# mstksg/tensor-ops

Measured on AMD Instinct MI355X. Metric: gradTOp steps/sec (ffLayer MNIST 784->256->10) + gmul TFLOP/s vs roofline, higher is better.
Workload: dtype f32

## Files before the change

### tensor-ops_amd/csrc/gemm_small.hip

```cpp
#include "common.hpp"

#include <type_traits>

namespace to {

typedef float f32x16 __attribute__((ext_vector_type(16)));

template <class S>
struct SmallArgsT {
  const S* A;
  const S* B;
  S* C;
  const S* Cin;
  int M, N, K;
  long a_sm, a_sk, b_sk, b_sn, c_sm;
  long a_sb, b_sb, c_sb;
  int a_vec, b_vec;
  unsigned a_bytes, b_bytes;
  int tiles_n;
  int tiles_m;
  int tile_order;
  int kper;
  S alpha, beta;
  const S* bias;
  const S* dact;
  int act;
  int dact_kind;
  S* rowsum;
  const S* rowsum_in;
  S rowsum_alpha;
  int rowsum_acc;
  int loss_rows;
  const S* target;
  S* loss_out;
  const S* tail_w;
  const S* tail_h;
  S* tail_out;
  int tail_n;
#ifdef TOPS_AB_KNOBS
  long long* dbg;
#endif
};

#ifdef TOPS_AB_KNOBS
#define SM_STAMP(i) do { if (stamp_on) g.dbg[i] = wall_clock64(); } while (0)
#else
#define SM_STAMP(i) do { } while (0)
#endif


template <class G>
__device__ __forceinline__ void tile_of(const G& g, int bid, int& tile_m, int& tile_n) {
  if (g.tile_order) {
    const int T = g.tiles_m * g.tiles_n, x = bid & 7, q = T >> 3, r = T & 7;
    bid = (x < r ? x * (q + 1) : r * (q + 1) + (x - r) * q) + (bid >> 3);
  }
  if (g.tile_order == 2) {
    tile_n = bid / g.tiles_m;
    tile_m = bid - tile_n * g.tiles_m;
  } else {
    tile_m = bid / g.tiles_n;
    tile_n = bid - tile_m * g.tiles_n;
  }
}

__device__ __forceinline__ float tanh_s(float x) { return tanhf(x); }
__device__ __forceinline__ double tanh_s(double x) { return tanh(x); }
__device__ __forceinline__ float exp_s(float x) { return expf(x); }
__device__ __forceinline__ double exp_s(double x) { return exp(x); }
__device__ __forceinline__ float log_s(float x) { return logf(x); }
__device__ __forceinline__ double log_s(double x) { return log(x); }
__device__ __forceinline__ float max_s(float a, float b) { return fmaxf(a, b); }
__device__ __forceinline__ double max_s(double a, double b) { return fmax(a, b); }

template <int OFF>
__device__ __forceinline__ float xor16(float x) {
  const int v = __float_as_int(x);
  if constexpr (OFF == 1) return __int_as_float(__builtin_amdgcn_update_dpp(v, v, 0xB1, 0xF, 0xF, false));
  else if constexpr (OFF == 2) return __int_as_float(__builtin_amdgcn_update_dpp(v, v, 0x4E, 0xF, 0xF, false));
  else if constexpr (OFF == 8) return __int_as_float(__builtin_amdgcn_update_dpp(v, v, 0x128, 0xF, 0xF, false));
  else {
    static_assert(OFF == 4, "xor 8, 4, 2 or 1");
    const int up = __builtin_amdgcn_update_dpp(v, v, 0x104, 0xF, 0x5, false);
    return __int_as_float(__builtin_amdgcn_update_dpp(up, v, 0x114, 0xF, 0xA, false));
  }
}
template <int OFF>
__device__ __forceinline__ double xor16(double x) { return __shfl_xor(x, OFF, 64); }

template <class S, int AMODE, int BMODE, int NW, int TS, int ONESHOT = 0, bool EXT = false, int PARTS = 0, bool STAG = false, int TAILK = 0>
__device__ __forceinline__ void gemm_small_body(const SmallArgsT<S>& g, const int bid, const long bz, S* ext_lds = nullptr,
                                                const int tid_in = -1) {
  constexpr int ES = (int)sizeof(S);
  static_assert(ES == 4 || TS == 16, "the fp64 matrix instruction is 16x16x4");
  constexpr int KG = (TS == 32) ? 2 : 4;
  constexpr int NR = (TS == 32) ? 16 : 4;
  constexpr int CK = 4 * KG;
  typedef S accv __attribute__((ext_vector_type(NR)));
  S (*red)[NR][64];
  S (*rsum)[64];
  S* dzs;
  if constexpr (EXT) {
    red = reinterpret_cast<S (*)[NR][64]>(ext_lds);
    rsum = reinterpret_cast<S (*)[64]>(ext_lds + NW * NR * 64);
    dzs = ext_lds + NW * NR * 64 + NW * 64;
  } else {
    __shared__ S red_s[NW][NR][64];
    __shared__ S rsum_s[NW][64];
    __shared__ S dzs_s[TS == 16 ? 16 * 17 : 1];
    red = red_s;
    rsum = rsum_s;
    dzs = dzs_s;
  }
  const int tid = tid_in >= 0 ? tid_in : (int)threadIdx.x, lane = tid & 63, wave = tid >> 6;
  const int l31 = lane & (TS - 1), half = lane / TS;
#ifdef TOPS_AB_KNOBS
  const bool stamp_on = g.dbg && bid == 0 && tid == 0;
#endif
  SM_STAMP(0);
  int tile_m, tile_n;
  tile_of(g, bid, tile_m, tile_n);
  const long m = (long)tile_m * TS + l31, n = (long)tile_n * TS + l31;
  const bool mv = m < g.M, nv = n < g.N;

  accv acc;
#pragma unroll
  for (int r = 0; r < NR; ++r) acc[r] = S(0);
  S asum = S(0);

  const int kbeg = wave * g.kper;
  int kend = kbeg + g.kper;
  if (kend > g.K) kend = g.K;

  constexpr int ST = ONESHOT ? ONESHOT : 4;
  S a0[ST][4], b0[ST][4];
  const __amdgpu_buffer_rsrc_t ra = __builtin_amdgcn_make_buffer_rsrc(
      const_cast<S*>(g.A), 0, g.a_bytes, 0x00020000);
  const __amdgpu_buffer_rsrc_t rb = __builtin_amdgcn_make_buffer_rsrc(
      const_cast<S*>(g.B), 0, g.b_bytes, 0x00020000);
  const int a_base = (int)((bz * g.a_sb + (mv ? m : 0) * g.a_sm) * ES);
  const int b_base = (int)((bz * g.b_sb + (nv ? n : 0) * g.b_sn) * ES);
  const int a_sk4 = (int)g.a_sk * ES, b_sk4 = (int)g.b_sk * ES;
  auto sel = [](bool ok, int off) { const int msk = -(int)ok; return (off & msk) | (0x7fffffff & ~msk); };
  typedef unsigned int u32x4 __attribute__((ext_vector_type(4)));
  typedef unsigned int u32x2 __attribute__((ext_vector_type(2)));
  auto ld1 = [&](__amdgpu_buffer_rsrc_t r, int off) -> S {
    if constexpr (ES == 4) {
      return __uint_as_float(__builtin_amdgcn_raw_buffer_load_b32(r, off, 0, 0));
    } else {
      const u32x2 v = __builtin_amdgcn_raw_buffer_load_b64(r, off, 0, 0);
      return __hiloint2double((int)v.y, (int)v.x);
    }
  };
  auto ld4 = [&](__amdgpu_buffer_rsrc_t r, bool ok, int off, S (&d)[4]) {
    if constexpr (ES == 4) {
      const u32x4 v = __builtin_amdgcn_raw_buffer_load_b128(r, sel(ok, off), 0, 0);
      d[0] = __uint_as_float(v.x); d[1] = __uint_as_float(v.y);
      d[2] = __uint_as_float(v.z); d[3] = __uint_as_float(v.w);
    } else {
      const u32x4 v = __builtin_amdgcn_raw_buffer_load_b128(r, sel(ok, off), 0, 0);
      const u32x4 w = __builtin_amdgcn_raw_buffer_load_b128(r, sel(ok, off + 16), 0, 0);
      d[0] = __hiloint2double((int)v.y, (int)v.x); d[1] = __hiloint2double((int)v.w, (int)v.z);
      d[2] = __hiloint2double((int)w.y, (int)w.x); d[3] = __hiloint2double((int)w.w, (int)w.z);
    }
  };
  auto load_stage = [&](S (&a)[ST][4], S (&b)[ST][4], int k0) {
#pragma unroll
    for (int c = 0; c < ST; ++c) {
      const int kb = k0 + CK * c + 4 * half;
      if (AMODE == 0 && g.a_vec) {
        ld4(ra, mv & (kb < kend), a_base + kb * ES, a[c]);
      } else {
#pragma unroll
        for (int j = 0; j < 4; ++j) a[c][j] = ld1(ra, sel(mv & (kb + j < kend), a_base + (kb + j) * a_sk4));
      }
      if (BMODE == 1 && g.b_vec) {
        ld4(rb, nv & (kb < kend), b_base + kb * ES, b[c]);
      } else {
#pragma unroll
        for (int j = 0; j < 4; ++j) b[c][j] = ld1(rb, sel(nv & (kb + j < kend), b_base + (kb + j) * b_sk4));
      }
    }
  };
  auto mma_stage = [&](const S (&a)[ST][4], const S (&b)[ST][4]) {
#pragma unroll
    for (int c = 0; c < ST; ++c)
#pragma unroll
      for (int j = 0; j < 4; ++j) {
        if constexpr (ES == 8) acc = __builtin_amdgcn_mfma_f64_16x16x4f64(a[c][j], b[c][j], acc, 0, 0, 0);
        else if constexpr (TS == 32) acc = __builtin_amdgcn_mfma_f32_32x32x2f32(a[c][j], b[c][j], acc, 0, 0, 0);
        else acc = __builtin_amdgcn_mfma_f32_16x16x4f32(a[c][j], b[c][j], acc, 0, 0, 0);
        asum += a[c][j];
      }
  };
  constexpr int CP = PARTS ? ST / PARTS : ST;
  static_assert(PARTS == 0 || (ONESHOT && ST % PARTS == 0), "PARTS divides the one-shot batch");
  auto load_part = [&](auto part, int k0) {
    constexpr int p = decltype(part)::value;
#pragma unroll
    for (int c = p * CP; c < (p + 1) * CP; ++c) {
      const int kb = k0 + CK * c + 4 * half;
      if (AMODE == 0 && g.a_vec) {
        ld4(ra, mv & (kb < kend), a_base + kb * ES, a0[c]);
      } else {
#pragma unroll
        for (int j = 0; j < 4; ++j) a0[c][j] = ld1(ra, sel(mv & (kb + j < kend), a_base + (kb + j) * a_sk4));
      }
      if (BMODE == 1 && g.b_vec) {
        ld4(rb, nv & (kb < kend), b_base + kb * ES, b0[c]);
      } else {
#pragma unroll
        for (int j = 0; j < 4; ++j) b0[c][j] = ld1(rb, sel(nv & (kb + j < kend), b_base + (kb + j) * b_sk4));
      }
      __builtin_amdgcn_sched_barrier(0);
    }
  };
  auto mma_part = [&](auto part) {
    constexpr int p = decltype(part)::value;
#pragma unroll
    for (int c = p * CP; c < (p + 1) * CP; ++c) {
#pragma unroll
      for (int j = 0; j < 4; ++j) {
        if constexpr (ES == 8) acc = __builtin_amdgcn_mfma_f64_16x16x4f64(a0[c][j], b0[c][j], acc, 0, 0, 0);
        else if constexpr (TS == 32) acc = __builtin_amdgcn_mfma_f32_32x32x2f32(a0[c][j], b0[c][j], acc, 0, 0, 0);
        else acc = __builtin_amdgcn_mfma_f32_16x16x4f32(a0[c][j], b0[c][j], acc, 0, 0, 0);
      }
      __builtin_amdgcn_sched_barrier(0);
#pragma unroll
      for (int j = 0; j < 4; ++j) asum += a0[c][j];
      __builtin_amdgcn_sched_barrier(0);
    }
  };
  auto row16 = [&](int kg, int r) { return ES == 8 ? kg + 4 * r : 4 * kg + r; };
  constexpr int NRW = (NR + NW - 1) / NW;
  S* Cb = g.C + bz * g.c_sb;
  const S* Ci = g.Cin ? g.Cin + bz * g.c_sb : nullptr;
  const S* Hd = g.dact ? g.dact + bz * g.c_sb : nullptr;
  S pf_ci[NRW], pf_hd[NRW], pf_bias = S(0);
  {
    const long col = (long)tile_n * TS + l31;
    if (g.bias && col < g.N) pf_bias = g.bias[col];
#pragma unroll
    for (int i = 0; i < NRW; ++i) {
      const int r = wave + i * NW;
      const int lrow = (TS == 32) ? (r & 3) + 8 * (r >> 2) + 4 * half : row16(half, r);
      const long row = (long)tile_m * TS + lrow;
      const bool ok = r < NR && row < g.M && col < g.N;
      pf_ci[i] = (Ci && ok) ? Ci[row * g.c_sm + col] : S(0);
      pf_hd[i] = (Hd && ok) ? Hd[row * g.c_sm + col] : S(0);
    }
  }
  constexpr int SK = CK * ST;
  SM_STAMP(1);
  if constexpr (ONESHOT) {
    if constexpr (PARTS == 0) {
      if (kbeg < kend) {
        load_stage(a0, b0, kbeg);
#ifdef TOPS_AB_KNOBS
        if (stamp_on) { SM_STAMP(2); __builtin_amdgcn_s_waitcnt(0x0F70); SM_STAMP(3); }
#endif
        mma_stage(a0, b0);
      }
    } else if (kbeg < kend) {
      if constexpr (STAG) {
        const int lvl = __builtin_amdgcn_readfirstlane(wave) >> 2;
        if (lvl == 0) __builtin_amdgcn_s_setprio(3);
        else if (lvl == 1) __builtin_amdgcn_s_setprio(2);
        else if (lvl == 2) __builtin_amdgcn_s_setprio(1);
      }
      load_part(std::integral_constant<int, 0>{}, kbeg);
      auto stage = [&](auto part) {
        constexpr int p = decltype(part)::value;
        if constexpr (p + 1 < PARTS) load_part(std::integral_constant<int, p + 1>{}, kbeg);
        if constexpr (STAG && p == (PARTS >= 2 ? PARTS - 2 : 0)) __builtin_amdgcn_s_setprio(0);
        __builtin_amdgcn_sched_barrier(0);
        if constexpr (p == 0) SM_STAMP(2);
        mma_part(part);
        __builtin_amdgcn_sched_barrier(0);
        if constexpr (p == 0) SM_STAMP(3);
      };
      stage(std::integral_constant<int, 0>{});
      if constexpr (PARTS > 1) stage(std::integral_constant<int, 1>{});
      if constexpr (PARTS > 2) stage(std::integral_constant<int, 2>{});
      if constexpr (PARTS > 3) stage(std::integral_constant<int, 3>{});
      if constexpr (PARTS > 4) {
        stage(std::integral_constant<int, 4>{});
        stage(std::integral_constant<int, 5>{});
        stage(std::integral_constant<int, 6>{});
        stage(std::integral_constant<int, 7>{});
      }
      static_assert(PARTS == 1 || PARTS == 2 || PARTS == 4 || PARTS == 8, "one, two, four or eight parts");
    }
  } else {
    S a1[ST][4], b1[ST][4];
    if (kbeg < kend) load_stage(a0, b0, kbeg);
    for (int k0 = kbeg; k0 < kend; k0 += 2 * SK) {
      if (k0 + SK < kend) load_stage(a1, b1, k0 + SK);
      mma_stage(a0, b0);
      if (k0 + SK < kend) {
        if (k0 + 2 * SK < kend) load_stage(a0, b0, k0 + 2 * SK);
        mma_stage(a1, b1);
      }
    }
  }

  S tl_bw[2][4], tl_hv[2][4];
  if constexpr (TS == 16) {
    if (g.loss_rows && g.tail_out) {
      const int l15 = lane & 15, kg = lane >> 4;
      const int ntiles = (g.tail_n + 15) / 16;
#pragma unroll
      for (int u = 0; u < 2; ++u) {
        const int t = wave + u * NW;
        const long col = (long)t * 16 + l15;
        const bool cv = t < ntiles && col < g.tail_n;
#pragma unroll
        for (int st = 0; st < 4; ++st) {
          const int k = 4 * st + kg;
          tl_bw[u][st] = (cv && k < g.N) ? g.tail_w[(long)k * g.tail_n + col] : S(0);
        }
#pragma unroll
        for (int r = 0; r < 4; ++r) {
          const long row = (long)tile_m * 16 + row16(kg, r);
          tl_hv[u][r] = (cv && row < g.M) ? g.tail_h[row * g.tail_n + col] : S(0);
        }
      }
    }
  }
#pragma unroll
  for (int r = 0; r < NR; ++r) red[wave][r][lane] = acc[r];
  rsum[wave][lane] = asum;
  SM_STAMP(4);
  __syncthreads();
  SM_STAMP(5);
  if (g.rowsum && tile_n == 0 && wave == 0 && lane < TS) {
    S v = S(0);
#pragma unroll
    for (int w = 0; w < NW; ++w)
#pragma unroll
      for (int q = 0; q < KG; ++q) v += rsum[w][lane + q * TS];
    const long row = (long)tile_m * TS + lane;
    if (row < g.M) g.rowsum[bz * g.M + row] = g.rowsum_acc ? g.rowsum_in[bz * g.M + row] + g.rowsum_alpha * v : v;
  }
#pragma unroll
  for (int i = 0; i < NRW; ++i) {
    const int r = wave + i * NW;
    if (r >= NR) break;
    S v = S(0);
#pragma unroll
    for (int w = 0; w < NW; ++w) v += red[w][r][lane];
    const int lrow = (TS == 32) ? (r & 3) + 8 * (r >> 2) + 4 * half : row16(half, r);
    const long row = (long)tile_m * TS + lrow;
    const long col = (long)tile_n * TS + l31;
    if constexpr (TS == 16) {
      if (g.loss_rows) {
        const bool valid = row < g.M && col < g.N;
        v = v * g.alpha + pf_bias;
        const S t = valid ? g.target[row * g.c_sm + col] : S(0);
        auto sum16 = [](S x) {
          x += xor16<8>(x); x += xor16<4>(x); x += xor16<2>(x); x += xor16<1>(x);
          return x;
        };
        S out, l;
        if (g.loss_rows == 1) {
          S mx = valid ? v : S(-INFINITY);
          mx = max_s(mx, xor16<8>(mx)); mx = max_s(mx, xor16<4>(mx));
          mx = max_s(mx, xor16<2>(mx)); mx = max_s(mx, xor16<1>(mx));
          const S e = valid ? exp_s(v - mx) : S(0);
          const S se = sum16(e), sy = sum16(t);
          const S pr = e / se;
          out = pr * sy - t;
          l = valid ? -t * log_s(pr) : S(0);
        } else {
          const S sg = S(1) / (S(1) + exp_s(-v));
          const S e = t - sg;
          out = S(-2) * e * sg * (S(1) - sg);
          l = valid ? e * e : S(0);
        }
        if (valid) Cb[row * g.c_sm + col] = out;
        if (g.tail_out) dzs[lrow * 17 + l31] = valid ? out : S(0);
        if (g.loss_out) {
          l = sum16(l);
          if (l31 == 0 && row < g.M) g.loss_out[row] = l;
        }
        continue;
      }
    }
    if (row < g.M && col < g.N) {
      v *= g.alpha;
      if (Ci) v += g.beta * pf_ci[i];
      v += pf_bias;
      if (g.act == 1) v = S(1) / (S(1) + exp_s(-v));
      else if (g.act == 2) v = tanh_s(v);
      if (Hd) {
        const S h = pf_hd[i];
        v *= g.dact_kind ? S(1) - h * h : h * (S(1) - h);
      }
      Cb[row * g.c_sm + col] = v;
    }
  }
  SM_STAMP(6);
  if constexpr (TS == 16) {
    if (g.loss_rows && g.tail_out) {
      __syncthreads();
      typedef S acc4 __attribute__((ext_vector_type(4)));
      const int l15 = lane & 15, kg = lane >> 4;
      const int ntiles = (g.tail_n + 15) / 16;
      acc4 acc2[2];
#pragma unroll
      for (int u = 0; u < 2; ++u)
#pragma unroll
        for (int r = 0; r < 4; ++r) acc2[u][r] = S(0);
#pragma unroll
      for (int st = 0; st < 4; ++st) {
        if (4 * st < g.N) {
          const S a = dzs[l15 * 17 + 4 * st + kg];
#pragma unroll
          for (int u = 0; u < 2; ++u) {
            if constexpr (ES == 8) acc2[u] = __builtin_amdgcn_mfma_f64_16x16x4f64(a, tl_bw[u][st], acc2[u], 0, 0, 0);
            else acc2[u] = __builtin_amdgcn_mfma_f32_16x16x4f32(a, tl_bw[u][st], acc2[u], 0, 0, 0);
          }
        }
      }
#pragma unroll
      for (int u = 0; u < 2; ++u) {
        const int t = wave + u * NW;
        const long col = (long)t * 16 + l15;
#pragma unroll
        for (int r = 0; r < 4; ++r) {
          const long row = (long)tile_m * 16 + row16(kg, r);
          if (t < ntiles && row < g.M && col < g.tail_n) {
            if constexpr (TAILK == ACT_KIND_TANH) g.tail_out[row * g.tail_n + col] = acc2[u][r] * tanh_dact(tl_hv[u][r]);
            else g.tail_out[row * g.tail_n + col] = acc2[u][r] * tl_hv[u][r] * (S(1) - tl_hv[u][r]);
          }
        }
      }
      SM_STAMP(7);
    }
  }
#ifdef TOPS_AB_KNOBS
  if (stamp_on) { __builtin_amdgcn_s_waitcnt(0); SM_STAMP(8); }
#endif
}

template <class S, int AMODE, int BMODE, int NW, int TS, int ONESHOT = 0, int TAILK = 0>
__global__ __launch_bounds__(NW * 64) void gemm_small_kernel(SmallArgsT<S> g) {
  gemm_small_body<S, AMODE, BMODE, NW, TS, ONESHOT, false, 0, false, TAILK>(g, (int)blockIdx.x, (long)blockIdx.z);
}

__global__ __launch_bounds__(8 * 64) void gemm_small_head_kernel(SmallArgsT<float> g) {
  g.a_vec = 1;
  g.b_vec = 1;
  gemm_small_body<float, 0, 1, 8, 16, 2>(g, (int)blockIdx.x, (long)blockIdx.z);
}
__global__ __launch_bounds__(8 * 64) void gemm_small_head_tanh_kernel(SmallArgsT<float> g) {
  g.a_vec = 1;
  g.b_vec = 1;
  gemm_small_body<float, 0, 1, 8, 16, 2, false, 0, false, ACT_KIND_TANH>(g, (int)blockIdx.x, (long)blockIdx.z);
}

template <class S, int A1, int B1, int NW1, int TS1, int OS1, int A2, int B2, int NW2, int TS2, int OS2, int P1 = 0, bool STAG1 = false>
__global__ __launch_bounds__((NW1 > NW2 ? NW1 : NW2) * 64) void gemm_small_pair_kernel(SmallArgsT<S> g1,
                                                                                         SmallArgsT<S> g2, int n1) {
  if ((int)blockIdx.x < n1) {
    if (NW1 < NW2 && (int)(threadIdx.x >> 6) >= NW1) return;
    gemm_small_body<S, A1, B1, NW1, TS1, OS1, false, P1, STAG1>(g1, (int)blockIdx.x, 0);
  } else {
    if (NW2 < NW1 && (int)(threadIdx.x >> 6) >= NW2) return;
    gemm_small_body<S, A2, B2, NW2, TS2, OS2>(g2, (int)blockIdx.x - n1, 0);
  }
}

struct ChainSync {
  unsigned* ctr;
  int* status;
  long long timeout;
  int dev;
};

__device__ __forceinline__ bool chain_barrier(const ChainSync& cs, int which, unsigned epoch) {
  __shared__ int ok;
  if (cs.dev == 1) {
    __syncthreads();
    return true;
  }
  if (cs.dev != 2) __builtin_amdgcn_fence(__ATOMIC_RELEASE, "agent");
  if (threadIdx.x == 0) ok = 1;
  __syncthreads();
  unsigned* flags = cs.ctr + which * 256;
  if (threadIdx.x == 0) __hip_atomic_store(flags + blockIdx.x, epoch, __ATOMIC_RELEASE, __HIP_MEMORY_SCOPE_AGENT);
  if (threadIdx.x < gridDim.x) {
    const long long t0 = wall_clock64();
    while (__hip_atomic_load(flags + threadIdx.x, __ATOMIC_RELAXED, __HIP_MEMORY_SCOPE_AGENT) < epoch) {
      if (wall_clock64() - t0 > cs.timeout) {
        ok = 0;
        *cs.status = 1 + which;
        break;
      }
      __builtin_amdgcn_s_sleep(1);
    }
  }
  __syncthreads();
  if (cs.dev != 2) __builtin_amdgcn_fence(__ATOMIC_ACQUIRE, "agent");
  return ok != 0;
}

struct ChainArgs {
  SmallArgsT<float> g[4];
  int nblk[2];
  int n1, n2;
  ChainSync cs;
};

__global__ __launch_bounds__(1024) void gemm_small_chain_kernel(ChainArgs c) {
  extern __shared__ __attribute__((aligned(16))) float chain_lds[];
  const unsigned epoch = __hip_atomic_load(c.cs.ctr + 512, __ATOMIC_RELAXED, __HIP_MEMORY_SCOPE_AGENT) + 1;
  const int bid = (int)blockIdx.x;
  if (bid < c.nblk[0]) gemm_small_body<float, 0, 1, 16, 32, 8, true>(c.g[0], bid, 0, chain_lds);
  if (!chain_barrier(c.cs, 0, epoch)) return;
  if (bid < c.nblk[1]) gemm_small_body<float, 0, 1, 16, 16, 8, true>(c.g[1], bid, 0, chain_lds);
  if (!chain_barrier(c.cs, 1, epoch)) return;
  if (bid == 0 && threadIdx.x == 0) __hip_atomic_store(c.cs.ctr + 512, epoch, __ATOMIC_RELAXED, __HIP_MEMORY_SCOPE_AGENT);
  if (bid < c.n1) gemm_small_body<float, 1, 0, 16, 32, 8, true>(c.g[2], bid, 0, chain_lds);
  else if (bid < c.n1 + c.n2) gemm_small_body<float, 1, 0, 16, 16, 8, true>(c.g[3], bid - c.n1, 0, chain_lds);
}

struct SeamArgs {
  SmallArgsT<float> fwd;
  SmallArgsT<float> head;
  unsigned* ctr;
  int mode;
  long long* dbg;
  int* status;
};

__global__ __launch_bounds__(1024) void gemm_small_seam_kernel(SeamArgs c) {
  extern __shared__ __attribute__((aligned(16))) float seam_lds[];
  __shared__ int seam_go;
  const int bid = (int)blockIdx.x;
  int tile_m, tile_n;
  tile_of(c.fwd, bid, tile_m, tile_n);
  unsigned* ctr = c.ctr + tile_m * 32;
  const bool stamp = c.dbg && tile_m == 0 && threadIdx.x == 0;
  long long t_start = 0, t_fwd = 0, t_stored = 0;
  if (stamp) t_start = wall_clock64();
  const unsigned base = ctr[1];
  gemm_small_body<float, 0, 1, 16, 32, 8, true>(c.fwd, bid, 0, seam_lds);
  if (stamp) t_fwd = wall_clock64();
  __builtin_amdgcn_s_waitcnt(0);
  __syncthreads();
  if (stamp) t_stored = wall_clock64();
  const unsigned ntile = (unsigned)c.fwd.tiles_n;
  if (c.mode == 2) {
    if (tile_n != (int)ntile - 1) {
      if (threadIdx.x == 0) __hip_atomic_fetch_add(ctr, 1u, __ATOMIC_RELAXED, __HIP_MEMORY_SCOPE_AGENT);
      return;
    }
    if (threadIdx.x == 0) {
      const long long t0 = wall_clock64();
      int ok = 1;
      while ((int)(__hip_atomic_load(ctr, __ATOMIC_RELAXED, __HIP_MEMORY_SCOPE_AGENT) - (base + ntile - 1u)) < 0) {
        if (wall_clock64() - t0 > 200000000LL) {
          ok = 0;
          if (c.status) *c.status = 1 + tile_m;
          break;
        }
        __builtin_amdgcn_s_sleep(1);
      }
      seam_go = ok;
      if (ok) ctr[1] = base + ntile - 1u;
    }
  } else {
    if (threadIdx.x == 0) {
      const unsigned seen = __hip_atomic_fetch_add(ctr, 1u, __ATOMIC_RELAXED, __HIP_MEMORY_SCOPE_AGENT);
      seam_go = (seen + 1u - base) == ntile;
      if (seam_go) ctr[1] = seen + 1u;
    }
  }
  __syncthreads();
  if (!seam_go) return;
  long long t_go = 0;
  if (stamp) t_go = wall_clock64();
  const int hw = (int)threadIdx.x >> 9;
  constexpr int HEAD_LDS = 8 * 4 * 64 + 8 * 64 + 16 * 17 + 16;
  gemm_small_body<float, 0, 1, 8, 16, 2, true>(c.head, 2 * tile_m + hw, 0, seam_lds + hw * HEAD_LDS, (int)threadIdx.x & 511);
  if (stamp) {
    c.dbg[0] = t_start; c.dbg[1] = t_fwd; c.dbg[2] = t_stored; c.dbg[3] = t_go; c.dbg[4] = wall_clock64();
  }
}

template <int AMODE, int BMODE, int NW, int ST, int D = 2>
__device__ __forceinline__ void gemm_small_f64_t32_body(const SmallArgsT<double>& g, const int bid, const long bz) {
  typedef double S;
  typedef double acc4 __attribute__((ext_vector_type(4)));
  constexpr int CK = 16, SK = ST * CK, NQ = 16;
  __shared__ S red[NW][NQ][64];
  __shared__ S rsum[NW][2][64];
  const int tid = threadIdx.x, lane = tid & 63, wave = tid >> 6;
  const int l15 = lane & 15, kg = lane >> 4;
  int tile_m, tile_n;
  tile_of(g, bid, tile_m, tile_n);
  long m[2], n[2];
  bool mv[2], nv[2];
#pragma unroll
  for (int h = 0; h < 2; ++h) {
    m[h] = (long)tile_m * 32 + 16 * h + l15;
    n[h] = (long)tile_n * 32 + 16 * h + l15;
    mv[h] = m[h] < g.M;
    nv[h] = n[h] < g.N;
  }
  acc4 acc[2][2];
#pragma unroll
  for (int i = 0; i < 2; ++i)
#pragma unroll
    for (int j = 0; j < 2; ++j) acc[i][j] = acc4{0.0, 0.0, 0.0, 0.0};
  S asum[2] = {0.0, 0.0};
  const int kbeg = wave * g.kper;
  int kend = kbeg + g.kper;
  if (kend > g.K) kend = g.K;

  const __amdgpu_buffer_rsrc_t ra = __builtin_amdgcn_make_buffer_rsrc(const_cast<S*>(g.A), 0, g.a_bytes, 0x00020000);
  const __amdgpu_buffer_rsrc_t rb = __builtin_amdgcn_make_buffer_rsrc(const_cast<S*>(g.B), 0, g.b_bytes, 0x00020000);
  int a_base[2], b_base[2];
#pragma unroll
  for (int h = 0; h < 2; ++h) {
    a_base[h] = (int)((bz * g.a_sb + (mv[h] ? m[h] : 0) * g.a_sm) * 8);
    b_base[h] = (int)((bz * g.b_sb + (nv[h] ? n[h] : 0) * g.b_sn) * 8);
  }
  const int a_sk8 = (int)g.a_sk * 8, b_sk8 = (int)g.b_sk * 8;
  auto sel = [](bool ok, int off) { const int msk = -(int)ok; return (off & msk) | (0x7fffffff & ~msk); };
  typedef unsigned int u32x4 __attribute__((ext_vector_type(4)));
  typedef unsigned int u32x2 __attribute__((ext_vector_type(2)));
  auto ld1 = [&](__amdgpu_buffer_rsrc_t r, int off) -> S {
    const u32x2 v = __builtin_amdgcn_raw_buffer_load_b64(r, off, 0, 0);
    return __hiloint2double((int)v.y, (int)v.x);
  };
  auto ld4 = [&](__amdgpu_buffer_rsrc_t r, bool ok, int off, S (&d)[4]) {
    const u32x4 v = __builtin_amdgcn_raw_buffer_load_b128(r, sel(ok, off), 0, 0);
    const u32x4 w = __builtin_amdgcn_raw_buffer_load_b128(r, sel(ok, off + 16), 0, 0);
    d[0] = __hiloint2double((int)v.y, (int)v.x); d[1] = __hiloint2double((int)v.w, (int)v.z);
    d[2] = __hiloint2double((int)w.y, (int)w.x); d[3] = __hiloint2double((int)w.w, (int)w.z);
  };
  auto load_stage = [&](S (&a)[2][ST][4], S (&b)[2][ST][4], int k0) {
#pragma unroll
    for (int c = 0; c < ST; ++c) {
      const int kb = k0 + CK * c + 4 * kg;
#pragma unroll
      for (int h = 0; h < 2; ++h) {
        if (AMODE == 0 && g.a_vec) {
          ld4(ra, mv[h] & (kb < kend), a_base[h] + kb * 8, a[h][c]);
        } else {
#pragma unroll
          for (int j = 0; j < 4; ++j) a[h][c][j] = ld1(ra, sel(mv[h] & (kb + j < kend), a_base[h] + (kb + j) * a_sk8));
        }
        if (BMODE == 1 && g.b_vec) {
          ld4(rb, nv[h] & (kb < kend), b_base[h] + kb * 8, b[h][c]);
        } else {
#pragma unroll
          for (int j = 0; j < 4; ++j) b[h][c][j] = ld1(rb, sel(nv[h] & (kb + j < kend), b_base[h] + (kb + j) * b_sk8));
        }
      }
    }
  };
  auto mma_stage = [&](const S (&a)[2][ST][4], const S (&b)[2][ST][4]) {
#pragma unroll
    for (int c = 0; c < ST; ++c)
#pragma unroll
      for (int j = 0; j < 4; ++j) {
#pragma unroll
        for (int i = 0; i < 2; ++i) {
#pragma unroll
          for (int q = 0; q < 2; ++q) acc[i][q] = __builtin_amdgcn_mfma_f64_16x16x4f64(a[i][c][j], b[q][c][j], acc[i][q], 0, 0, 0);
          asum[i] += a[i][c][j];
        }
      }
  };
  constexpr int NQW = (NQ + NW - 1) / NW;
  S* Cb = g.C + bz * g.c_sb;
  const S* Ci = g.Cin ? g.Cin + bz * g.c_sb : nullptr;
  const S* Hd = g.dact ? g.dact + bz * g.c_sb : nullptr;
  S pf_ci[NQW], pf_hd[NQW], pf_bias[NQW];
#pragma unroll
  for (int u = 0; u < NQW; ++u) {
    const int q = wave + u * NW;
    const long row = (long)tile_m * 32 + 16 * (q >> 3) + kg + 4 * (q & 3);
    const long col = (long)tile_n * 32 + 16 * ((q >> 2) & 1) + l15;
    const bool ok = q < NQ && row < g.M && col < g.N;
    pf_ci[u] = (Ci && ok) ? Ci[row * g.c_sm + col] : 0.0;
    pf_hd[u] = (Hd && ok) ? Hd[row * g.c_sm + col] : 0.0;
    pf_bias[u] = (g.bias && ok) ? g.bias[col] : 0.0;
  }
  {
    S a[D][2][ST][4], b[D][2][ST][4];
    const int nst = (kend - kbeg + SK - 1) / SK;
#pragma unroll
    for (int d = 0; d < D - 1; ++d)
      if (d < nst) load_stage(a[d], b[d], kbeg + d * SK);
    for (int s0 = 0; s0 < nst; s0 += D) {
#pragma unroll
      for (int d = 0; d < D; ++d) {
        const int st = s0 + d;
        if (st < nst) {
          if (st + D - 1 < nst) load_stage(a[(d + D - 1) % D], b[(d + D - 1) % D], kbeg + (st + D - 1) * SK);
          mma_stage(a[d], b[d]);
        }
      }
    }
  }
#pragma unroll
  for (int i = 0; i < 2; ++i)
#pragma unroll
    for (int j = 0; j < 2; ++j)
#pragma unroll
      for (int r = 0; r < 4; ++r) red[wave][(i * 2 + j) * 4 + r][lane] = acc[i][j][r];
  rsum[wave][0][lane] = asum[0];
  rsum[wave][1][lane] = asum[1];
  __syncthreads();
  if (g.rowsum && tile_n == 0 && wave == 0 && lane < 32) {
    const int h = lane >> 4;
    S v = 0.0;
#pragma unroll
    for (int w = 0; w < NW; ++w)
#pragma unroll
      for (int q = 0; q < 4; ++q) v += rsum[w][h][l15 + 16 * q];
    const long row = (long)tile_m * 32 + lane;
    if (row < g.M) g.rowsum[bz * g.M + row] = g.rowsum_acc ? g.rowsum_in[bz * g.M + row] + g.rowsum_alpha * v : v;
  }
#pragma unroll
  for (int u = 0; u < NQW; ++u) {
    const int q = wave + u * NW;
    if (q >= NQ) break;
    S v = 0.0;
#pragma unroll
    for (int w = 0; w < NW; ++w) v += red[w][q][lane];
    const long row = (long)tile_m * 32 + 16 * (q >> 3) + kg + 4 * (q & 3);
    const long col = (long)tile_n * 32 + 16 * ((q >> 2) & 1) + l15;
    if (row < g.M && col < g.N) {
      v *= g.alpha;
      if (Ci) v += g.beta * pf_ci[u];
      v += pf_bias[u];
      if (g.act == 1) v = 1.0 / (1.0 + exp(-v));
      else if (g.act == 2) v = tanh(v);
      if (Hd) v *= g.dact_kind ? 1.0 - pf_hd[u] * pf_hd[u] : pf_hd[u] * (1.0 - pf_hd[u]);
      Cb[row * g.c_sm + col] = v;
    }
  }
}

template <int AMODE, int BMODE, int NW, int ST, int D = 2>
__global__ __launch_bounds__(NW * 64) void gemm_small_f64_t32_kernel(SmallArgsT<double> g) {
  gemm_small_f64_t32_body<AMODE, BMODE, NW, ST, D>(g, (int)blockIdx.x, (long)blockIdx.z);
}

template <int A1, int B1, int A2, int B2>
__global__ __launch_bounds__(512) void gemm_small_pair_f64_kernel(SmallArgsT<double> g1, SmallArgsT<double> g2, int n1) {
  if ((int)blockIdx.x < n1) gemm_small_f64_t32_body<A1, B1, 8, 1>(g1, (int)blockIdx.x, 0);
  else gemm_small_body<double, A2, B2, 8, 16, 8>(g2, (int)blockIdx.x - n1, 0);
}

bool gemm_small_fuses_loss(const GemmProblem& p) {
  const int64_t tiles64 = ((p.M + 63) / 64) * ((p.N + 63) / 64) * p.batch;
  return gemm_small_can(p) && tiles64 < 200 && p.N <= 16 && p.batch == 1 && p.beta == 0.0 && !p.dact && p.act == 0;
}

bool gemm_small_fuses_tail(const GemmProblem& p, int64_t tail_n) {
  return gemm_small_fuses_loss(p) && tail_n <= 256 && (p.K + 15) / 16 >= 8;
}

bool gemm_small_can(const GemmProblem& p) {
  if (p.dtype != TO_F32 && p.dtype != TO_F64) return false;
  if (p.reduce_batch) return false;
  if (p.batch > 65535) return false;
  if (p.M < 1 || p.N < 1 || p.K < 1) return false;
  const int64_t es = p.dtype == TO_F64 ? 8 : 4;
  auto span = [es](int64_t nb, int64_t sb, int64_t n0, int64_t s0, int64_t n1, int64_t s1) {
    return ((nb - 1) * sb + (n0 - 1) * s0 + (n1 - 1) * s1 + 1) * es;
  };
  if (span(p.batch, p.a_sb, p.M, p.a_sm, p.K, p.a_sk) >= (1LL << 31) ||
      span(p.batch, p.b_sb, p.N, p.b_sn, p.K, p.b_sk) >= (1LL << 31))
    return false;
  if (p.a_sm < 0 || p.a_sk < 0 || p.b_sk < 0 || p.b_sn < 0) return false;
  const int64_t tiles16 = ((p.M + 15) / 16) * ((p.N + 15) / 16) * p.batch;
  return tiles16 <= 65535;
}

bool gemm_small_applicable(const GemmProblem& p) {
  if (!gemm_small_can(p)) return false;
  const int64_t tiles64 = ((p.M + 63) / 64) * ((p.N + 63) / 64) * p.batch;
  return tiles64 < 200 && p.M * p.N >= 256;
}

static int pick_tile_order(const GemmProblem& p, int ts, int tiles_m, int tiles_n) {
  static const int enable = [] { const char* e = ab_getenv("TOPS_SMALL_XCD"); return e ? atoi(e) : 1; }();
  const long T = (long)tiles_m * tiles_n;
  if (!enable || T < 16) return 0;
  if (enable == 2 || enable == 3) return enable - 1;
  const long run = (T + 7) / 8;
  const double a_panel = (double)ts * p.K, b_panel = (double)ts * p.K;
  const double row_cost = (double)((run + tiles_n - 1) / tiles_n + 1) * a_panel + (double)(run < tiles_n ? run + 1 : tiles_n) * b_panel;
  const double col_cost = (double)((run + tiles_m - 1) / tiles_m + 1) * b_panel + (double)(run < tiles_m ? run + 1 : tiles_m) * a_panel;
  return col_cost < row_cost ? 2 : 1;
}

template <class S, int NW, int TS, int ONESHOT = 0, int TAILK = 0>
static void launch_nw(SmallArgsT<S>& g, const GemmProblem& p, int amode, int bmode, hipStream_t s) {
  constexpr int CK = (TS == 32) ? 8 : 16;
  const int chunks = (int)((p.K + CK - 1) / CK);
  g.kper = ((chunks + NW - 1) / NW) * CK;
  const int tiles_m = (int)((p.M + TS - 1) / TS);
  g.tiles_n = (int)((p.N + TS - 1) / TS);
  g.tiles_m = tiles_m;
  g.tile_order = pick_tile_order(p, TS, g.tiles_m, g.tiles_n);
  dim3 grid(tiles_m * g.tiles_n, 1, (unsigned)p.batch), block(NW * 64);
  switch (amode * 2 + bmode) {
    case 0: launch_k((gemm_small_kernel<S, 0, 0, NW, TS, ONESHOT, TAILK>), grid, block, 0, s, g); break;
    case 1: launch_k((gemm_small_kernel<S, 0, 1, NW, TS, ONESHOT, TAILK>), grid, block, 0, s, g); break;
    case 2: launch_k((gemm_small_kernel<S, 1, 0, NW, TS, ONESHOT, TAILK>), grid, block, 0, s, g); break;
    default: launch_k((gemm_small_kernel<S, 1, 1, NW, TS, ONESHOT, TAILK>), grid, block, 0, s, g); break;
  }
}

#ifdef TOPS_AB_KNOBS
static long long* small_stamps(int which) {
  static const int want = [] { const char* e = ab_getenv("TOPS_SMALL_STAMPS"); return e ? atoi(e) : 0; }();
  if (!want || want != which) return nullptr;
  static long long* buf = [] {
    long long* p = nullptr;
    if (hipHostMalloc(&p, 16 * sizeof(long long), hipHostMallocMapped) != hipSuccess) return (long long*)nullptr;
    for (int i = 0; i < 16; ++i) p[i] = 0;
    static long long* keep = p;
    atexit([] {
      static const char* names[9] = {"entry", "set-up done", "operand batch issued", "operand batch landed", "MFMAs done, partial in LDS",
                                     "all partials there (barrier)", "reduced + epilogue / loss head, stores issued", "tail done", "stores acknowledged"};
      std::fprintf(stderr, "[small stamps %d] tile 0, thread 0, us since its workgroup began:", want);
      for (int i = 1; i < 9; ++i)
        if (keep[i]) std::fprintf(stderr, "\n  %6.2f  %s", (keep[i] - keep[0]) * 0.01, names[i]);
      std::fprintf(stderr, "\n");
    });
    return p;
  }();
  long long* dev = nullptr;
  if (buf && hipHostGetDevicePointer(reinterpret_cast<void**>(&dev), buf, 0) != hipSuccess) dev = nullptr;
  return dev;
}
#endif

struct SmallPlan {
  int ts, nw, os;
  int amode, bmode;
  bool f64_t32;
};

template <class S>
static SmallPlan plan_small(const GemmProblem& p, SmallArgsT<S>& g) {
  constexpr bool F64 = sizeof(S) == 8;
  g = SmallArgsT<S>{};
  g.A = (const S*)p.A; g.B = (const S*)p.B; g.C = (S*)p.C;
  g.Cin = (p.beta != 0.0) ? (const S*)p.Cin : nullptr;
  g.M = (int)p.M; g.N = (int)p.N; g.K = (int)p.K;
  g.a_sm = p.a_sm; g.a_sk = p.a_sk; g.b_sk = p.b_sk; g.b_sn = p.b_sn; g.c_sm = p.c_sm;
  g.a_sb = p.a_sb; g.b_sb = p.b_sb; g.c_sb = p.c_sb;
  g.alpha = (S)p.alpha; g.beta = (S)p.beta;
  g.bias = (const S*)p.bias; g.dact = (const S*)p.dact; g.act = p.act; g.dact_kind = p.dact_kind;
  g.rowsum = (S*)p.rowsum;
  g.rowsum_acc = p.rowsum_acc ? 1 : 0; g.rowsum_alpha = (S)p.rowsum_alpha;
  g.rowsum_in = p.rowsum_in ? (const S*)p.rowsum_in : (const S*)p.rowsum;
  g.loss_rows = p.loss_rows; g.target = (const S*)p.target; g.loss_out = (S*)p.loss_out;
  g.tail_w = (const S*)p.tail_w; g.tail_h = (const S*)p.tail_h;
  g.tail_out = p.loss_rows ? (S*)p.tail_out : nullptr; g.tail_n = p.tail_n;
  TO_CHECK(!g.tail_out || p.tail_n <= 256, TO_ERR_ARG, "fused tail: at most 256 columns (gemm_small_fuses_tail)");
  auto al16 = [](const void* q) { return (reinterpret_cast<uintptr_t>(q) & 15u) == 0; };
  auto eff = [](int64_t stride, int64_t extent) { return extent == 1 ? (int64_t)0 : stride; };
  SmallPlan c{};
  c.amode = (p.a_sk == 1) ? 0 : 1;
  c.bmode = (p.b_sk == 1 && p.b_sn != 1) ? 1 : 0;
  constexpr int64_t VE = 16 / (int64_t)sizeof(S);
  g.a_vec = c.amode == 0 && p.K % 4 == 0 && al16(p.A) && eff(p.a_sm, p.M) % VE == 0 && eff(p.a_sb, p.batch) % VE == 0;
  g.b_vec = c.bmode == 1 && p.K % 4 == 0 && al16(p.B) && eff(p.b_sn, p.N) % VE == 0 && eff(p.b_sb, p.batch) % VE == 0;
  g.a_bytes = (unsigned)(((p.batch - 1) * eff(p.a_sb, p.batch) + (p.M - 1) * eff(p.a_sm, p.M) +
                          (p.K - 1) * eff(p.a_sk, p.K) + 1) * (int64_t)sizeof(S));
  g.b_bytes = (unsigned)(((p.batch - 1) * eff(p.b_sb, p.batch) + (p.N - 1) * eff(p.b_sn, p.N) +
                          (p.K - 1) * eff(p.b_sk, p.K) + 1) * (int64_t)sizeof(S));
  static const int force_nw = [] { const char* e = ab_getenv("TOPS_SMALL_NW"); return e ? atoi(e) : 0; }();
  const bool t16 = F64 || (p.M <= 16 || p.N <= 16 || p.K <= 32);
  const int ts = t16 ? 16 : 32, ck = t16 ? 16 : 8;
  const int64_t tiles = ((p.M + ts - 1) / ts) * ((p.N + ts - 1) / ts) * p.batch;
  const int64_t chunks = (p.K + ck - 1) / ck;
  int nw = 8;
  while (nw > 1 && (tiles * nw > 4096 || chunks / nw < 4)) nw >>= 1;
  if (force_nw) nw = force_nw;
  if (g.tail_out) {
    TO_CHECK(t16 && chunks >= 8, TO_ERR_ARG, "fused tail: shape not eligible (gemm_small_fuses_tail)");
    nw = 8;
  }
  c.ts = ts;
  c.nw = nw;
  c.os = 0;
  static const int oneshot = [] { const char* e = ab_getenv("TOPS_SMALL_ONESHOT"); return e ? atoi(e) : 1; }();
  if (!F64 && oneshot && !force_nw && !t16 && tiles * 16 <= 4096 && chunks > 88 && chunks <= 128) {
    c.nw = 16;
    c.os = 8;
  }
  static const int oneshot8 = [] { const char* e = ab_getenv("TOPS_SMALL_ONESHOT8"); return e ? atoi(e) : 1; }();
  if (oneshot8 && !force_nw && t16 && nw == 8 && chunks > 32 && chunks <= 64 && !g.tail_out) c.os = 8;
  static const int f64_t32 = [] { const char* e = ab_getenv("TOPS_SMALL_F64_T32"); return e ? atoi(e) : 1; }();
  if (F64 && f64_t32 && !force_nw && !g.loss_rows && p.M > 16 && p.N > 16 && p.K >= 128) {
    const int64_t t32 = ((p.M + 31) / 32) * ((p.N + 31) / 32) * p.batch;
    int w = 8;
    while (w > 2 && (t32 * w > 4096 || chunks / w < 4)) w >>= 1;
    c.f64_t32 = true;
    c.ts = 32;
    c.nw = w;
    c.os = w == 8 ? 1 : 2;
    g.kper = (int)(((chunks + w - 1) / w) * 16);
    g.tiles_n = (int)((p.N + 31) / 32);
    g.tiles_m = (int)((p.M + 31) / 32);
    g.tile_order = pick_tile_order(p, 32, g.tiles_m, g.tiles_n);
    return c;
  }
  g.kper = (int)(((chunks + c.nw - 1) / c.nw) * ck);
  g.tiles_n = (int)((p.N + c.ts - 1) / c.ts);
  g.tiles_m = (int)((p.M + c.ts - 1) / c.ts);
  g.tile_order = pick_tile_order(p, c.ts, g.tiles_m, g.tiles_n);
  return c;
}

template <class S>
static void launch_small_t(const GemmProblem& p, hipStream_t s) {
  constexpr bool F64 = sizeof(S) == 8;
  SmallArgsT<S> g;
  const SmallPlan c = plan_small<S>(p, g);
#ifdef TOPS_AB_KNOBS
  if (g.loss_rows) g.dbg = small_stamps(2);
#endif
  const int amode = c.amode, bmode = c.bmode;
  if constexpr (F64) {
    if (c.f64_t32) {
      const int tiles_m = (int)((p.M + 31) / 32);
      dim3 grid(tiles_m * g.tiles_n, 1, (unsigned)p.batch), block(c.nw * 64);
#define TOPS_F64_T32(AM, BM)                                                                              \
  switch (c.nw * 10 + c.os) {                                                                             \
    case 22: launch_k((gemm_small_f64_t32_kernel<AM, BM, 2, 2>), grid, block, 0, s, g); break;  \
    case 42: launch_k((gemm_small_f64_t32_kernel<AM, BM, 4, 2>), grid, block, 0, s, g); break;  \
    default: launch_k((gemm_small_f64_t32_kernel<AM, BM, 8, 1>), grid, block, 0, s, g); break;  \
  }
      switch (amode * 2 + bmode) {
        case 0: TOPS_F64_T32(0, 0) break;
        case 1: TOPS_F64_T32(0, 1) break;
        case 2: TOPS_F64_T32(1, 0) break;
        default: TOPS_F64_T32(1, 1) break;
      }
#undef TOPS_F64_T32
      TO_HIP(hipGetLastError());
      count_launch();
      return;
    }
  }
  static const int head_lean = [] { const char* e = ab_getenv("TOPS_SMALL_HEAD_LEAN"); return e ? atoi(e) : 1; }();
  const bool tanh_tail = g.tail_out && p.tail_kind == ACT_KIND_TANH;
  bool lean = false;
  if constexpr (!F64)
    lean = head_lean && g.loss_rows && c.ts == 16 && c.nw == 8 && c.os == 0 && amode == 0 && bmode == 1 && g.a_vec && g.b_vec &&
           p.K <= 8 * 2 * 16;
  if (lean) {
    if constexpr (!F64) {
      const dim3 grid((unsigned)(g.tiles_m * g.tiles_n), 1, (unsigned)p.batch), block(8 * 64);
      if (tanh_tail) launch_k(gemm_small_head_tanh_kernel, grid, block, 0, s, g);
      else launch_k(gemm_small_head_kernel, grid, block, 0, s, g);
    }
  } else if (tanh_tail) {
    TO_CHECK(c.ts == 16 && c.nw == 8 && c.os == 0, TO_ERR_STATE, "internal: fused tail outside its configuration");
    launch_nw<S, 8, 16, 0, ACT_KIND_TANH>(g, p, amode, bmode, s);
  } else if (c.os == 8 && c.nw == 16) {
    if constexpr (!F64) launch_nw<S, 16, 32, 8>(g, p, amode, bmode, s);
  } else if (c.os == 8) {
    launch_nw<S, 8, 16, 8>(g, p, amode, bmode, s);
  } else if (c.ts == 16) {
    switch (c.nw) {
      case 1: launch_nw<S, 1, 16>(g, p, amode, bmode, s); break;
      case 2: launch_nw<S, 2, 16>(g, p, amode, bmode, s); break;
      case 4: launch_nw<S, 4, 16>(g, p, amode, bmode, s); break;
      default: launch_nw<S, 8, 16>(g, p, amode, bmode, s); break;
    }
  } else {
    if constexpr (!F64) {
      switch (c.nw) {
        case 1: launch_nw<S, 1, 32>(g, p, amode, bmode, s); break;
        case 2: launch_nw<S, 2, 32>(g, p, amode, bmode, s); break;
        case 4: launch_nw<S, 4, 32>(g, p, amode, bmode, s); break;
        default: launch_nw<S, 8, 32>(g, p, amode, bmode, s); break;
      }
    }
  }
  TO_HIP(hipGetLastError());
  count_launch();
}

static int* g_chain_status = nullptr;

bool launch_gemm_small_chain(const GemmProblem& pa, const GemmProblem& pb, const GemmProblem& pc1, const GemmProblem& pc2,
                             hipStream_t s) {
  static const int enable = [] { const char* e = ab_getenv("TOPS_STEP_CHAIN"); return e ? atoi(e) : 0; }();
  if (!enable) return false;
  if (pb.tail_out && pb.tail_kind) return false;
  const GemmProblem* ps[4] = {&pa, &pb, &pc1, &pc2};
  for (const GemmProblem* p : ps)
    if (p->dtype != TO_F32 || p->batch != 1 || !gemm_small_can(*p)) return false;
  ChainArgs c{};
  const SmallPlan ca = plan_small<float>(pa, c.g[0]);
  if (!(ca.ts == 32 && ca.nw == 16 && ca.os == 8 && ca.amode == 0 && ca.bmode == 1) || c.g[0].loss_rows) return false;
  const SmallPlan cb = plan_small<float>(pb, c.g[1]);
  if (!(cb.ts == 16 && cb.amode == 0 && cb.bmode == 1 && !cb.f64_t32) || !c.g[1].loss_rows) return false;
  const SmallPlan c1 = plan_small<float>(pc1, c.g[2]);
  if (!(c1.ts == 32 && c1.nw == 16 && c1.os == 8 && c1.amode == 1 && c1.bmode == 0) || c.g[2].loss_rows) return false;
  const SmallPlan c2 = plan_small<float>(pc2, c.g[3]);
  if (!(c2.ts == 16 && c2.amode == 1 && c2.bmode == 0) || c.g[3].loss_rows) return false;
  auto sixteen = [](const GemmProblem& p, SmallArgsT<float>& g) {
    const int64_t chunks = (p.K + 15) / 16;
    if (chunks > 128) return false;
    g.kper = (int)(((chunks + 15) / 16) * 16);
    return true;
  };
  if (!sixteen(pb, c.g[1]) || !sixteen(pc2, c.g[3])) return false;
  if (c.g[1].tail_out && c.g[1].tail_n > 256) return false;
  c.nblk[0] = (int)((pa.M + 31) / 32) * c.g[0].tiles_n;
  c.nblk[1] = (int)((pb.M + 15) / 16) * c.g[1].tiles_n;
  c.n1 = (int)((pc1.M + 31) / 32) * c.g[2].tiles_n;
  c.n2 = (int)((pc2.M + 15) / 16) * c.g[3].tiles_n;
  const int grid = std::max(std::max(c.nblk[0], c.nblk[1]), c.n1 + c.n2);
  if (grid > 256 || grid < 1) return false;
  constexpr size_t lds = (16 * 16 * 64 + 16 * 64 + 16 * 17 + 16) * sizeof(float);
  static unsigned* ctr = nullptr;
  static int *status = nullptr, *status_dev = nullptr;
  static int resident = -1;
  if (resident < 0) {
    int per_cu = 0;
    hipDeviceProp_t prop;
    if (hipFuncSetAttribute(reinterpret_cast<const void*>(gemm_small_chain_kernel), hipFuncAttributeMaxDynamicSharedMemorySize,
                            (int)lds) != hipSuccess ||
        hipOccupancyMaxActiveBlocksPerMultiprocessor(&per_cu, gemm_small_chain_kernel, 1024, lds) != hipSuccess ||
        hipGetDeviceProperties(&prop, rt().device) != hipSuccess) {
      (void)hipGetLastError();
      resident = 0;
    } else {
      resident = per_cu * prop.multiProcessorCount;
    }
    if (resident >= 256) {
      TO_HIP(hipMalloc(&ctr, 4096));
      TO_HIP(hipMemset(ctr, 0, 4096));
      TO_HIP(hipHostMalloc(&status, sizeof(int), hipHostMallocMapped));
      *status = 0;
      TO_HIP(hipHostGetDevicePointer(reinterpret_cast<void**>(&status_dev), status, 0));
    }
  }
  if (resident < grid || !ctr) return false;
  if (*status != 0) return false;
  c.cs.ctr = ctr;
  c.cs.status = status_dev;
  static const double timeout_s = [] { const char* e = ab_getenv("TOPS_CHAIN_TIMEOUT_S"); return e ? atof(e) : 1.0; }();
  c.cs.timeout = (long long)(timeout_s * 100e6);
  g_chain_status = status;
  static const int dev = [] { const char* e = ab_getenv("TOPS_CHAIN_DEV"); return e ? atoi(e) : 0; }();
  c.cs.dev = dev;
  launch_k(gemm_small_chain_kernel, dim3(grid), dim3(1024), lds, s, c);
  TO_HIP(hipGetLastError());
  count_launch();
  return true;
}

int gemm_small_chain_status() { return g_chain_status ? *g_chain_status : 0; }

static unsigned* g_seam_ctr = nullptr;
static int *g_seam_status = nullptr, *g_seam_status_dev = nullptr;
static bool g_seam_disabled = false;
int gemm_small_seam_status() { return g_seam_status ? *g_seam_status : 0; }
int gemm_small_seam_take_failure() {
  const int st = gemm_small_seam_status();
  if (st) {
    g_seam_disabled = true;
    *g_seam_status = 0;
  }
  return st;
}

void gemm_small_seam_init() {
  if (g_seam_ctr) return;
  if (!xcd_placement_probe()) return;
  if (hipMalloc(&g_seam_ctr, 4096 * sizeof(unsigned)) != hipSuccess) {
    g_seam_ctr = nullptr;
    (void)hipGetLastError();
    return;
  }
  if (hipHostMalloc(&g_seam_status, sizeof(int), hipHostMallocMapped) == hipSuccess) {
    *g_seam_status = 0;
    if (hipHostGetDevicePointer(reinterpret_cast<void**>(&g_seam_status_dev), g_seam_status, 0) != hipSuccess) g_seam_status_dev = nullptr;
  }
  (void)hipGetLastError();
  if (hipMemset(g_seam_ctr, 0, 4096 * sizeof(unsigned)) != hipSuccess ||
      hipFuncSetAttribute(reinterpret_cast<const void*>(gemm_small_seam_kernel), hipFuncAttributeMaxDynamicSharedMemorySize,
                          (int)((16 * 16 * 64 + 16 * 64 + 16 * 17 + 16) * sizeof(float))) != hipSuccess) {
    (void)hipGetLastError();
    (void)hipFree(g_seam_ctr);
    g_seam_ctr = nullptr;
  }
}

bool launch_gemm_small_seam(const GemmProblem& pf, const GemmProblem& ph, hipStream_t s) {
  if (ph.tail_out && ph.tail_kind) return false;
  if (launch_gemm_t32_head(pf, ph, s)) return true;
  static const int enable = [] { const char* e = getenv("TOPS_STEP_SEAM"); const int v = e ? atoi(e) : 0; return v == 1 || v == 2 ? v : 0; }();
  if (!enable || g_seam_disabled || gemm_small_seam_status() != 0) return false;
  if (pf.dtype != TO_F32 || ph.dtype != TO_F32 || pf.batch != 1 || ph.batch != 1) return false;
  if (!gemm_small_can(pf) || !gemm_small_can(ph) || !ph.loss_rows || pf.loss_rows) return false;
  if (ph.A != pf.C || ph.M != pf.M || ph.K != pf.N || ph.a_sk != 1 || ph.a_sm != pf.c_sm) return false;
  if (pf.rowsum || pf.dact || pf.beta != 0.0 || ph.beta != 0.0) return false;
  SeamArgs c{};
  const SmallPlan cf = plan_small<float>(pf, c.fwd);
  if (!(cf.ts == 32 && cf.nw == 16 && cf.os == 8 && cf.amode == 0 && cf.bmode == 1)) return false;
  const SmallPlan ch = plan_small<float>(ph, c.head);
  if (!(ch.ts == 16 && ch.nw == 8 && ch.amode == 0 && ch.bmode == 1 && !ch.f64_t32) || c.head.tiles_n != 1) return false;
  if (ph.K > 8 * 2 * 16) return false;
  c.head.kper = (int)((((ph.K + 15) / 16 + 7) / 8) * 16);
  c.head.tile_order = 0;
  const int T = c.fwd.tiles_m * c.fwd.tiles_n;
  if (T % 8 != 0 || (T / 8) % c.fwd.tiles_n != 0 || c.fwd.tiles_m > 128) return false;
  c.fwd.tile_order = 1;
  if (!g_seam_ctr) return false;
  c.ctr = g_seam_ctr;
  c.mode = enable == 2 ? 2 : 1;
  c.status = g_seam_status_dev;
  static long long* dbg = [] {
    long long* p = nullptr;
    if (ab_getenv("TOPS_SEAM_STAMPS") && hipHostMalloc(&p, 8 * sizeof(long long), hipHostMallocMapped) == hipSuccess) {
      for (int i = 0; i < 8; ++i) p[i] = 0;
      static long long* keep = p;
      atexit([] {
        std::fprintf(stderr, "[seam] row block 0's head (us since its workgroup began): forward done %.2f, stores in L2 %.2f, "
                             "all tiles arrived %.2f, head done %.2f\n",
                     (keep[1] - keep[0]) * 0.01, (keep[2] - keep[0]) * 0.01, (keep[3] - keep[0]) * 0.01, (keep[4] - keep[0]) * 0.01);
      });
      return p;
    }
    return (long long*)nullptr;
  }();
  c.dbg = dbg;
  constexpr size_t lds = (16 * 16 * 64 + 16 * 64 + 16 * 17 + 16) * sizeof(float);
  launch_k(gemm_small_seam_kernel, dim3(T), dim3(1024), lds, s, c);
  TO_HIP(hipGetLastError());
  count_launch();
  return true;
}

void launch_gemm_small(const GemmProblem& p, hipStream_t s) {
  if (gemm_t32_applicable(p)) {
    launch_gemm_t32(p, s);
    return;
  }
  if (p.dtype == TO_F64) launch_small_t<double>(p, s);
  else launch_small_t<float>(p, s);
}

constexpr int SMALL_PAIR_PARTS = 8;
constexpr bool SMALL_PAIR_STAG = false;

bool launch_gemm_small_pair(const GemmProblem& p1, const GemmProblem& p2, hipStream_t s, bool dry) {
  static const int enable = [] { const char* e = ab_getenv("TOPS_SMALL_PAIR"); return e ? atoi(e) : 1; }();
  if (!enable || p1.dtype != p2.dtype || p1.batch != 1 || p2.batch != 1) return false;
  if (launch_gemm_t32_pair(p1, p2, s, dry)) return true;
  if (!gemm_small_can(p1) || !gemm_small_can(p2)) return false;
  if (p1.dtype == TO_F64) {
    SmallArgsT<double> g1, g2;
    const SmallPlan c1 = plan_small<double>(p1, g1), c2 = plan_small<double>(p2, g2);
    if (!(c1.f64_t32 && c1.nw == 8 && c1.os == 1 && c1.amode == 1 && c1.bmode == 0)) return false;
    if (!(!c2.f64_t32 && c2.ts == 16 && c2.nw == 8 && c2.os == 8 && c2.amode == 1 && c2.bmode == 0)) return false;
    if (g1.loss_rows || g2.loss_rows) return false;
    if (dry) return true;
    const int n1 = (int)((p1.M + 31) / 32) * g1.tiles_n, n2 = (int)((p2.M + 15) / 16) * g2.tiles_n;
    launch_k((gemm_small_pair_f64_kernel<1, 0, 1, 0>), dim3(n1 + n2), dim3(512), 0, s, g1, g2, n1);
    TO_HIP(hipGetLastError());
    count_launch();
    return true;
  }
  SmallArgsT<float> g1, g2;
  const SmallPlan c1 = plan_small<float>(p1, g1), c2 = plan_small<float>(p2, g2);
#ifdef TOPS_AB_KNOBS
  g1.dbg = small_stamps(1);
  g2.dbg = small_stamps(3);
#endif
  if (c1.ts == 16 && c1.nw == 1 && c1.os == 0 && c1.amode == 1 && c1.bmode == 0 && !c1.f64_t32 &&
      c2.ts == 16 && c2.nw == 1 && c2.os == 0 && c2.amode == 1 && c2.bmode == 0 && !c2.f64_t32 && !g1.loss_rows && !g2.loss_rows) {
    const long t1 = (long)g1.tiles_m * g1.tiles_n, t2 = (long)g2.tiles_m * g2.tiles_n;
    if (t1 + t2 > 65535) return false;
    if (dry) return true;
    launch_k((gemm_small_pair_kernel<float, 1, 0, 1, 16, 0, 1, 0, 1, 16, 0>), dim3((unsigned)(t1 + t2)), dim3(64), 0, s, g1, g2, (int)t1);
    TO_HIP(hipGetLastError());
    count_launch();
    return true;
  }
  if (!(c1.ts == 32 && c1.nw == 16 && c1.os == 8 && c1.amode == 1 && c1.bmode == 0)) return false;
  if (!(c2.ts == 16 && c2.nw == 8 && c2.os == 8 && c2.amode == 1 && c2.bmode == 0)) return false;
  if (g1.loss_rows || g2.loss_rows) return false;
  if (dry) return true;
  const int n1 = (int)((p1.M + 31) / 32) * g1.tiles_n, n2 = (int)((p2.M + 15) / 16) * g2.tiles_n;
  dim3 grid(n1 + n2), block(1024);
#define TOPS_PAIR(P, ST) launch_k((gemm_small_pair_kernel<float, 1, 0, 16, 32, 8, 1, 0, 8, 16, 8, P, ST>), grid, block, 0, s, g1, g2, n1)
#ifdef TOPS_AB_KNOBS
  static const int parts = [] { const char* e = ab_getenv("TOPS_SMALL_PARTS"); return e ? atoi(e) : SMALL_PAIR_PARTS; }();
  static const int stag = [] { const char* e = ab_getenv("TOPS_SMALL_STAGGER"); return e ? atoi(e) : (int)SMALL_PAIR_STAG; }();
  switch (parts * 2 + (stag ? 1 : 0)) {
    case 0: TOPS_PAIR(0, false); break;
    case 2: TOPS_PAIR(1, false); break;
    case 3: TOPS_PAIR(1, true); break;
    case 4: TOPS_PAIR(2, false); break;
    case 5: TOPS_PAIR(2, true); break;
    case 8: TOPS_PAIR(4, false); break;
    case 9: TOPS_PAIR(4, true); break;
    case 16: TOPS_PAIR(8, false); break;
    case 17: TOPS_PAIR(8, true); break;
    default: TO_CHECK(false, TO_ERR_ARG, "TOPS_SMALL_PARTS is 0, 1, 2, 4 or 8 (TOPS_SMALL_STAGGER needs parts >= 1)");
  }
#else
  TOPS_PAIR(SMALL_PAIR_PARTS, SMALL_PAIR_STAG);
#endif
#undef TOPS_PAIR
  TO_HIP(hipGetLastError());
  count_launch();
  return true;
}

}
```

### tensor-ops_amd/csrc/gemm_t32.hip

```cpp
#include <cstdio>
#include <type_traits>

#include "common.hpp"

namespace to {

typedef float f32x16 __attribute__((ext_vector_type(16)));
typedef float f32x4 __attribute__((ext_vector_type(4)));

struct T32Args {
  const float* A;
  const float* B;
  float* C;
  const float* Cin;
  const float* bias;
  const float* dact;
  float* rowsum;
  const float* rowsum_in;
  unsigned long long* dbg;
  long a_sx, b_sx;
  long c_sm;
  int M, N, K;
  int tiles_m, tiles_n;
  int gm, gn;
  int act, dact_kind;
  int rowsum_acc;
  int pd;
  float alpha, beta;
  float rowsum_alpha;
};

__device__ __attribute__((aligned(16))) float g_t32_zero[4] = {0.f, 0.f, 0.f, 0.f};

constexpr int T32_BK = 32, T32_NS = 2, T32_NW = 4;
constexpr int T32_CTR = 4096;
constexpr int T32_STAGE = 2 * 32 * T32_BK;
constexpr int T32_WAVE = T32_NS * T32_STAGE;

__device__ __forceinline__ bool t32_tile_of(int tiles_m, int tiles_n, int gm, int gn, int bid, int& tm, int& tn) {
  const int x = bid & 7, local = bid >> 3, xm = x / gn, xn = x - xm * gn;
  const int r0 = tiles_m * xm / gm, r1 = tiles_m * (xm + 1) / gm, c0 = tiles_n * xn / gn, c1 = tiles_n * (xn + 1) / gn;
  const int w = c1 - c0;
  if (w <= 0 || local >= (r1 - r0) * w) return false;
  tm = r0 + local / w;
  tn = c0 + local - (local / w) * w;
  return true;
}

__device__ __forceinline__ int t32_key(int x) { return (x >> 1) & 7; }

template <bool AKC, bool BKC, bool ARAG = false, bool WT = false, int NW = T32_NW, int NS = T32_NS, bool EARLY = false, bool REGU = false>
__device__ __forceinline__ int gemm_t32_body(const T32Args& g, const int bid, float* smem) {
  static_assert(!REGU || (NW == 8 && NS == 1 && EARLY && !ARAG), "the register unit belongs to the eight-wave, one-stage, early-DMA form");
  constexpr int WAVE_F = NS * T32_STAGE;
  static_assert(WAVE_F >= 1024 + 64, "a wave's stage memory holds its partial tile and its row sums");
  static_assert(!ARAG || !AKC, "the dword form is for a row-contiguous A");
  constexpr int NA = ARAG ? 16 : 4, PER = NA + 4;
  const int tid = threadIdx.x, lane = tid & 63;
  const int wave = __builtin_amdgcn_readfirstlane(tid >> 6);
  const int l31 = lane & 31, half = lane >> 5;
  unsigned long long* const dbg = (g.dbg && tid == 0 && (bid == 0 || bid == (int)gridDim.x - 1)) ? g.dbg + (bid == 0 ? 0 : 8) : nullptr;
  auto stamp = [&](int i) { if (dbg) dbg[i] = __builtin_amdgcn_s_memrealtime(); };
#ifdef TOPS_AB_KNOBS
  unsigned long long* const wdbg = (g.dbg && lane == 0 && wave < 8 && (bid == 0 || bid == (int)gridDim.x - 1)) ? g.dbg + 16 + (bid == 0 ? 0 : 16) + 2 * wave : nullptr;
#define T32_WSTAMP(i) do { if (wdbg) wdbg[i] = __builtin_amdgcn_s_memrealtime(); } while (0)
#else
#define T32_WSTAMP(i) do { } while (0)
#endif
  int tile_m, tile_n;
  if (!t32_tile_of(g.tiles_m, g.tiles_n, g.gm, g.gn, bid, tile_m, tile_n)) return -1;
  stamp(0);
  const int m0 = tile_m * 32, n0 = tile_n * 32;

  const int erow = tid >> 3, ec4 = (tid & 7) * 4;
  const long grow = m0 + erow, gcol = n0 + ec4;
  const bool evalid = (NW == 4 || tid < 256) && grow < g.M && gcol < g.N;
  f32x4 pf_ci = {0.f, 0.f, 0.f, 0.f}, pf_hd = {0.f, 0.f, 0.f, 0.f}, pf_bias = {0.f, 0.f, 0.f, 0.f};
  auto prefetch_epilogue = [&] {
    if (evalid) {
      if (g.Cin) pf_ci = *reinterpret_cast<const f32x4*>(g.Cin + grow * g.c_sm + gcol);
      if (g.dact) pf_hd = *reinterpret_cast<const f32x4*>(g.dact + grow * g.c_sm + gcol);
      if (g.bias) pf_bias = *reinterpret_cast<const f32x4*>(g.bias + gcol);
    }
  };
  if constexpr (!EARLY) prefetch_epilogue();

  const int U = (g.K + 15) / 16;
  const int k0 = (int)((long)U * wave / NW) * 16;
  int k1 = (int)((long)U * (wave + 1) / NW) * 16;
  if (k1 > g.K) k1 = g.K;
  int kd = k1;
  bool ru = false;
  if constexpr (REGU) {
    const int nU = (k1 - k0 + 15) / 16;
    ru = (nU & 1) != 0;
    if (ru) kd = k0 + (nU - 1) * 16;
  }
  const int nC = kd > k0 ? (kd - k0 + T32_BK - 1) / T32_BK : 0;

  typedef __attribute__((address_space(3))) void* lptr_t;
  float* wsm = smem + wave * WAVE_F;
  const unsigned lds_w = __builtin_amdgcn_readfirstlane((unsigned)(unsigned long)(lptr_t)wsm);

  const int lr = lane >> 3, ls = lane & 7;
  unsigned oa[4], ob[4];
  bool xa_ok = true, xb_ok = true;
#pragma unroll
  for (int p = 0; p < 4; ++p) {
    if constexpr (AKC) {
      long x = m0 + 8 * p + lr;
      if (x >= g.M) x = g.M - 1;
      oa[p] = (unsigned)((x * g.a_sx + 4 * (ls ^ t32_key(8 * p + lr))) * 4);
    } else {
      oa[p] = (unsigned)(((long)(8 * p + lr) * g.a_sx + m0 + 4 * ls) * 4);
    }
    if constexpr (BKC) {
      long x = n0 + 8 * p + lr;
      if (x >= g.N) x = g.N - 1;
      ob[p] = (unsigned)((x * g.b_sx + 4 * (ls ^ t32_key(8 * p + lr))) * 4);
    } else {
      ob[p] = (unsigned)(((long)(8 * p + lr) * g.b_sx + n0 + 4 * ls) * 4);
    }
  }
  if constexpr (!AKC) xa_ok = m0 + 4 * ls + 3 < g.M;
  if constexpr (!BKC) xb_ok = n0 + 4 * ls + 3 < g.N;
  const bool interior = !ARAG && (AKC || m0 + 32 <= g.M) && (BKC || n0 + 32 <= g.N);
  const long step_a = AKC ? T32_BK * 4L : T32_BK * g.a_sx * 4L, step_b = BKC ? T32_BK * 4L : T32_BK * g.b_sx * 4L;
  const char* sa = reinterpret_cast<const char*>(g.A) + (AKC ? (long)k0 * 4 : (long)k0 * g.a_sx * 4);
  const char* sb = reinterpret_cast<const char*>(g.B) + (BKC ? (long)k0 * 4 : (long)k0 * g.b_sx * 4);

#define T32_DMA(OFF, BASE) asm volatile("global_load_lds_dwordx4 %0, %1 offset:0" ::"v"(OFF), "s"(BASE) : "memory")
#define T32_DMA_V(PTR) asm volatile("global_load_lds_dwordx4 %0, off offset:0" ::"v"(PTR) : "memory")
  const long a_sx_l = g.a_sx;
  const int M_l = g.M;
  auto issue = [&, a_sx_l, M_l](int c) {
    const int seq = c;
    const int kc = k0 + c * T32_BK;
    const unsigned st = lds_w + (unsigned)(seq % NS) * (T32_STAGE * 4);
    const char* ba = sa + (long)c * step_a;
    const char* bb = sb + (long)c * step_b;
    const bool full = kc + T32_BK <= kd;
    if (full && interior) {
#pragma unroll
      for (int p = 0; p < 4; ++p) {
        asm volatile("s_mov_b32 m0, %0\n\ts_nop 0" ::"s"(st + p * 1024) : "memory");
        T32_DMA(oa[p], ba);
      }
#pragma unroll
      for (int p = 0; p < 4; ++p) {
        asm volatile("s_mov_b32 m0, %0\n\ts_nop 0" ::"s"(st + 4096 + p * 1024) : "memory");
        T32_DMA(ob[p], bb);
      }
    } else {
      const char* zero = reinterpret_cast<const char*>(g_t32_zero);
      if constexpr (ARAG) {
#pragma unroll
        for (int e = 0; e < 16; ++e) {
          const int kl = 2 * e + half;
          const bool ok = kc + kl < kd && m0 + l31 < M_l;
          const char* src = ok ? ba + ((long)kl * a_sx_l + m0 + l31) * 4 : zero;
          asm volatile("s_mov_b32 m0, %0\n\ts_nop 0" ::"s"(st + e * 256) : "memory");
          asm volatile("global_load_lds_dword %0, off offset:0" ::"v"(src) : "memory");
        }
      } else {
#pragma unroll
        for (int p = 0; p < 4; ++p) {
          const bool ok = AKC ? (kc + 4 * (ls ^ t32_key(8 * p + lr)) < kd) : (kc + 8 * p + lr < kd && xa_ok);
          const char* src = ok ? ba + oa[p] : zero;
          asm volatile("s_mov_b32 m0, %0\n\ts_nop 0" ::"s"(st + p * 1024) : "memory");
          T32_DMA_V(src);
        }
      }
#pragma unroll
      for (int p = 0; p < 4; ++p) {
        const bool ok = BKC ? (kc + 4 * (ls ^ t32_key(8 * p + lr)) < kd) : (kc + 8 * p + lr < kd && xb_ok);
        const char* src = ok ? bb + ob[p] : zero;
        asm volatile("s_mov_b32 m0, %0\n\ts_nop 0" ::"s"(st + 4096 + p * 1024) : "memory");
        T32_DMA_V(src);
      }
    }
  };
#undef T32_DMA
#undef T32_DMA_V

  f32x16 acc;
#pragma unroll
  for (int r = 0; r < 16; ++r) acc[r] = 0.f;
  float asum = 0.f;
  const bool want_rs = g.rowsum != nullptr && tile_n == 0;

  const int PD = g.pd < NS ? g.pd : NS;
  const int pro = nC < PD ? nC : PD;
  f32x4 ua4[2], ub4[2];
  float ua1[8], ub1[8];
  if constexpr (REGU) {
    if (ru) {
      const float* zero = g_t32_zero;
#pragma unroll
      for (int i = 0; i < 2; ++i) {
        const int kq = kd + 4 * (2 * i + half);
        if constexpr (AKC) {
          long x = m0 + l31;
          if (x >= g.M) x = g.M - 1;
          const float* src = kq < k1 ? g.A + x * g.a_sx + kq : zero;
          asm volatile("global_load_dwordx4 %0, %1, off" : "=&v"(ua4[i]) : "v"(src) : "memory");
        } else {
#pragma unroll
          for (int j = 0; j < 4; ++j) {
            const float* src = (kq + j < k1 && m0 + l31 < g.M) ? g.A + (long)(kq + j) * g.a_sx + m0 + l31 : zero;
            asm volatile("global_load_dword %0, %1, off" : "=&v"(ua1[4 * i + j]) : "v"(src) : "memory");
          }
        }
        if constexpr (BKC) {
          long x = n0 + l31;
          if (x >= g.N) x = g.N - 1;
          const float* src = kq < k1 ? g.B + x * g.b_sx + kq : zero;
          asm volatile("global_load_dwordx4 %0, %1, off" : "=&v"(ub4[i]) : "v"(src) : "memory");
        } else {
#pragma unroll
          for (int j = 0; j < 4; ++j) {
            const float* src = (kq + j < k1 && n0 + l31 < g.N) ? g.B + (long)(kq + j) * g.b_sx + n0 + l31 : zero;
            asm volatile("global_load_dword %0, %1, off" : "=&v"(ub1[4 * i + j]) : "v"(src) : "memory");
          }
        }
      }
    }
    __builtin_amdgcn_sched_barrier(0);
  }
  if constexpr (EARLY) {
    if (pro > 0) issue(0);
    __builtin_amdgcn_sched_barrier(0);
    if constexpr (REGU) {
      if (ru) {
        if (pro > 0) asm volatile("s_waitcnt vmcnt(%0)" ::"n"(PER) : "memory");
        else asm volatile("s_waitcnt vmcnt(0)" ::: "memory");
        float fu[8], gu[8];
        if constexpr (AKC) {
          asm volatile("" : "+v"(ua4[0]), "+v"(ua4[1]) :: "memory");
#pragma unroll
          for (int i = 0; i < 2; ++i) { fu[4 * i] = ua4[i].x; fu[4 * i + 1] = ua4[i].y; fu[4 * i + 2] = ua4[i].z; fu[4 * i + 3] = ua4[i].w; }
        } else {
          asm volatile("" : "+v"(ua1[0]), "+v"(ua1[1]), "+v"(ua1[2]), "+v"(ua1[3]), "+v"(ua1[4]), "+v"(ua1[5]), "+v"(ua1[6]), "+v"(ua1[7]) :: "memory");
#pragma unroll
          for (int q = 0; q < 8; ++q) fu[q] = ua1[q];
        }
        if constexpr (BKC) {
          asm volatile("" : "+v"(ub4[0]), "+v"(ub4[1]) :: "memory");
#pragma unroll
          for (int i = 0; i < 2; ++i) { gu[4 * i] = ub4[i].x; gu[4 * i + 1] = ub4[i].y; gu[4 * i + 2] = ub4[i].z; gu[4 * i + 3] = ub4[i].w; }
        } else {
          asm volatile("" : "+v"(ub1[0]), "+v"(ub1[1]), "+v"(ub1[2]), "+v"(ub1[3]), "+v"(ub1[4]), "+v"(ub1[5]), "+v"(ub1[6]), "+v"(ub1[7]) :: "memory");
#pragma unroll
          for (int q = 0; q < 8; ++q) gu[q] = ub1[q];
        }
        __builtin_amdgcn_sched_barrier(0);
#pragma unroll
        for (int q = 0; q < 8; ++q) {
          acc = __builtin_amdgcn_mfma_f32_32x32x2f32(fu[q], gu[q], acc, 0, 0, 0);
          if (want_rs) asum += fu[q];
        }
      }
      __builtin_amdgcn_sched_barrier(0);
    }
    prefetch_epilogue();
    __builtin_amdgcn_sched_barrier(0);
    for (int c = 1; c < pro; ++c) issue(c);
  } else {
    for (int c = 0; c < pro; ++c) issue(c);
  }
  stamp(1);

  auto wait_landed = [&](int c) {
    const int newer = (nC - 1 - c) < (PD - 1) ? (nC - 1 - c) : (PD - 1);
    static_assert(3 * PER <= 63, "vmcnt is six bits");
    if (newer >= 3) asm volatile("s_waitcnt vmcnt(%0)" ::"n"(3 * PER) : "memory");
    else if (newer == 2) asm volatile("s_waitcnt vmcnt(%0)" ::"n"(2 * PER) : "memory");
    else if (newer == 1) asm volatile("s_waitcnt vmcnt(%0)" ::"n"(PER) : "memory");
    else asm volatile("s_waitcnt vmcnt(0)" ::: "memory");
  };
  auto steps_of = [&](int c) { return (kd - (k0 + c * T32_BK)) > 16 ? 4 : 2; };
  auto read_frags = [&](int c, float (&fa)[16], float (&fb)[16]) {
    const float* sp = wsm + (c % NS) * T32_STAGE;
    const int nI = steps_of(c);
#pragma unroll
    for (int i = 0; i < 4; ++i) {
      if (i < nI) {
        if constexpr (AKC) {
          const f32x4 v = *reinterpret_cast<const f32x4*>(sp + l31 * 32 + 4 * ((2 * i + half) ^ t32_key(l31)));
          fa[4 * i] = v.x; fa[4 * i + 1] = v.y; fa[4 * i + 2] = v.z; fa[4 * i + 3] = v.w;
        } else {
#pragma unroll
          for (int j = 0; j < 4; ++j) fa[4 * i + j] = sp[(4 * (2 * i + half) + j) * 32 + l31];
        }
        if constexpr (BKC) {
          const f32x4 v = *reinterpret_cast<const f32x4*>(sp + 1024 + l31 * 32 + 4 * ((2 * i + half) ^ t32_key(l31)));
          fb[4 * i] = v.x; fb[4 * i + 1] = v.y; fb[4 * i + 2] = v.z; fb[4 * i + 3] = v.w;
        } else {
#pragma unroll
          for (int j = 0; j < 4; ++j) fb[4 * i + j] = sp[1024 + (4 * (2 * i + half) + j) * 32 + l31];
        }
      }
    }
  };
  auto mma = [&](int c, const float (&fa)[16], const float (&fb)[16]) {
    const int nI = steps_of(c);
#pragma unroll
    for (int i = 0; i < 4; ++i) {
      if (i < nI) {
#pragma unroll
        for (int j = 0; j < 4; ++j) {
          acc = __builtin_amdgcn_mfma_f32_32x32x2f32(fa[4 * i + j], fb[4 * i + j], acc, 0, 0, 0);
          if (want_rs) asum += fa[4 * i + j];
        }
      }
    }
  };
  float fa[16], fb[16];
  for (int c = 0; c < nC; ++c) {
    wait_landed(c);
    if (c == 0) stamp(2);
    read_frags(c, fa, fb);
    asm volatile("s_waitcnt lgkmcnt(0)" ::: "memory");
    __builtin_amdgcn_sched_barrier(0);
    if (c + PD < nC) issue(c + PD);
    __builtin_amdgcn_sched_barrier(0);
    mma(c, fa, fb);
  }
  asm volatile("s_waitcnt vmcnt(0)" ::: "memory");
  stamp(3);
  T32_WSTAMP(0);

#pragma unroll
  for (int r = 0; r < 16; ++r) wsm[((r & 3) + 8 * (r >> 2) + 4 * half) * 32 + l31] = acc[r];
  if (want_rs) wsm[1024 + lane] = asum;
  T32_WSTAMP(1);
  __syncthreads();
  stamp(4);
  f32x4 s = {0.f, 0.f, 0.f, 0.f};
  if (NW == 4 || tid < 256) {
    s = *reinterpret_cast<const f32x4*>(smem + erow * 32 + ec4);
#pragma unroll
    for (int w = 1; w < NW; ++w) s += *reinterpret_cast<const f32x4*>(smem + w * WAVE_F + erow * 32 + ec4);
  }
  if (evalid) {
    f32x4 v = s * g.alpha;
    if (g.Cin) v += pf_ci * g.beta;
    if (g.bias) v += pf_bias;
    if (g.act == 1) {
      v.x = 1.f / (1.f + __expf(-v.x)); v.y = 1.f / (1.f + __expf(-v.y));
      v.z = 1.f / (1.f + __expf(-v.z)); v.w = 1.f / (1.f + __expf(-v.w));
    } else if (g.act == 2) {
      v.x = tanhf(v.x); v.y = tanhf(v.y); v.z = tanhf(v.z); v.w = tanhf(v.w);
    }
    if (g.dact) {
      if (g.dact_kind == 0) v *= pf_hd * (1.f - pf_hd);
      else v *= 1.f - pf_hd * pf_hd;
    }
    if constexpr (WT) {
      typedef unsigned int u32x4 __attribute__((ext_vector_type(4)));
      const u32x4 u = {__float_as_uint(v.x), __float_as_uint(v.y), __float_as_uint(v.z), __float_as_uint(v.w)};
      float* dst = g.C + grow * g.c_sm + gcol;
      asm volatile("global_store_dwordx4 %0, %1, off sc0 sc1" ::"v"(dst), "v"(u) : "memory");
    } else {
      *reinterpret_cast<f32x4*>(g.C + grow * g.c_sm + gcol) = v;
    }
  }
  if (want_rs && tid < 32) {
    const long m = m0 + tid;
    if (m < g.M) {
      float t = 0.f;
#pragma unroll
      for (int w = 0; w < NW; ++w) t += smem[w * WAVE_F + 1024 + tid] + smem[w * WAVE_F + 1024 + 32 + tid];
      if (g.rowsum_acc) g.rowsum[m] = (g.rowsum_in ? g.rowsum_in[m] : g.rowsum[m]) + g.rowsum_alpha * t;
      else g.rowsum[m] = t;
    }
  }
  stamp(5);
#undef T32_WSTAMP
  return tile_m;
}

struct T32HeadArgs {
  const float* W2;
  const float* bias2;
  const float* target;
  float* dz;
  float* loss_out;
  float* tail_out;
  unsigned* ctr;
  int* status;
  long w_sn, dz_sm;
  int N2, loss_rows;
  float alpha2;
};

__global__ __launch_bounds__(256) void gemm_t32_head_kernel(T32Args g, T32HeadArgs h) {
  extern __shared__ __attribute__((aligned(1024))) float t32_smem[];
  const int tid = threadIdx.x, lane = tid & 63;
  const int wave = __builtin_amdgcn_readfirstlane(tid >> 6);
  const unsigned long long t_entry = g.dbg ? __builtin_amdgcn_s_memrealtime() : 0ull;
  int tile_m, tile_n;
  if (!t32_tile_of(g.tiles_m, g.tiles_n, g.gm, g.gn, (int)blockIdx.x, tile_m, tile_n)) return;
  const long grow = (long)tile_m * 32 + 4 * tile_n + wave;
  const bool rv = grow < g.M;
  f32x4 w4[16];
#pragma unroll
  for (int n = 0; n < 16; ++n) {
    w4[n] = f32x4{0.f, 0.f, 0.f, 0.f};
    if (n < h.N2) w4[n] = *reinterpret_cast<const f32x4*>(h.W2 + (long)n * h.w_sn + 4 * lane);
  }
  const float b_l = (lane < h.N2 && h.bias2) ? h.bias2[lane] : 0.f;
  const float t_l = (lane < h.N2 && rv) ? h.target[grow * h.dz_sm + lane] : 0.f;

  gemm_t32_body<true, true, false, true>(g, (int)blockIdx.x, t32_smem);

  unsigned long long* const hd = (g.dbg && tid == 0 && blockIdx.x == 0) ? g.dbg + 8 : nullptr;
  asm volatile("s_waitcnt vmcnt(0)" ::: "memory");
  __syncthreads();
  __shared__ int gave_up;
  if (tid == 0) {
    unsigned* arrive = h.ctr + tile_m;
    __hip_atomic_fetch_add(arrive, 1u, __ATOMIC_RELAXED, __HIP_MEMORY_SCOPE_AGENT);
    if (hd) { hd[0] = t_entry; hd[1] = __builtin_amdgcn_s_memrealtime(); hd[7] = 1; }
    const unsigned long long t0 = __builtin_amdgcn_s_memrealtime();
    int bad = 0;
    while (__hip_atomic_load(arrive, __ATOMIC_RELAXED, __HIP_MEMORY_SCOPE_AGENT) < (unsigned)g.tiles_n) {
      __builtin_amdgcn_s_sleep(2);
      if (__builtin_amdgcn_s_memrealtime() - t0 > 200000000ull) {
        bad = 1;
        break;
      }
    }
    gave_up = bad;
    if (bad && h.status) *h.status = tile_m + 1;
  }
  __syncthreads();
  if (gave_up) return;
  if (hd) hd[2] = __builtin_amdgcn_s_memrealtime();

  typedef unsigned int u32x4 __attribute__((ext_vector_type(4)));
  f32x4 h4 = {0.f, 0.f, 0.f, 0.f};
  if (rv) {
    u32x4 u;
    const float* src = g.C + grow * g.c_sm + 4 * lane;
    asm volatile("global_load_dwordx4 %0, %1, off sc0 sc1\n\ts_waitcnt vmcnt(0)" : "=v"(u) : "v"(src) : "memory");
    h4 = f32x4{__uint_as_float(u.x), __uint_as_float(u.y), __uint_as_float(u.z), __uint_as_float(u.w)};
  }
  float z[16];
#pragma unroll
  for (int n = 0; n < 16; ++n) {
    z[n] = 0.f;
    if (n < h.N2) {
      z[n] = h4.x * w4[n].x + h4.y * w4[n].y + h4.z * w4[n].z + h4.w * w4[n].w;
#pragma unroll
      for (int off = 1; off < 64; off <<= 1) z[n] += __shfl_xor(z[n], off, 64);
    }
  }
  float v = -INFINITY;
#pragma unroll
  for (int n = 0; n < 16; ++n)
    if (n < h.N2 && lane == n) v = z[n] * h.alpha2 + b_l;
  auto sum16 = [](float x) {
#pragma unroll
    for (int off = 8; off > 0; off >>= 1) x += __shfl_xor(x, off, 64);
    return x;
  };
  const bool lv = lane < h.N2;
  float out_l, loss_l;
  if (h.loss_rows == 1) {
    float mx = v;
#pragma unroll
    for (int off = 8; off > 0; off >>= 1) mx = fmaxf(mx, __shfl_xor(mx, off, 64));
    const float e = lv ? expf(v - mx) : 0.f;
    const float se = sum16(e), sy = sum16(t_l);
    const float pr = e / se;
    out_l = lv ? pr * sy - t_l : 0.f;
    loss_l = lv ? -t_l * logf(pr) : 0.f;
  } else {
    const float sg = 1.f / (1.f + expf(-v));
    const float e = t_l - sg;
    out_l = lv ? -2.f * e * sg * (1.f - sg) : 0.f;
    loss_l = lv ? e * e : 0.f;
  }
  if (rv) {
    if (lv) h.dz[grow * h.dz_sm + lane] = out_l;
    if (h.loss_out) {
      const float l = sum16(loss_l);
      if (lane == 0) h.loss_out[grow] = l;
    }
  }
  if (hd) hd[3] = __builtin_amdgcn_s_memrealtime();
  if (h.tail_out) {
    f32x4 a = {0.f, 0.f, 0.f, 0.f};
#pragma unroll
    for (int n = 0; n < 16; ++n)
      if (n < h.N2) {
        const float d = __shfl(out_l, n, 64);
        a += w4[n] * d;
      }
    if (rv) *reinterpret_cast<f32x4*>(h.tail_out + grow * 256 + 4 * lane) = a * h4 * (1.f - h4);
  }
  if (hd) hd[4] = __builtin_amdgcn_s_memrealtime();
  __syncthreads();
  if (tid == 0) {
    unsigned* leave = h.ctr + T32_CTR + tile_m;
    const unsigned seen = __hip_atomic_fetch_add(leave, 1u, __ATOMIC_RELAXED, __HIP_MEMORY_SCOPE_AGENT);
    if (seen == (unsigned)(g.tiles_n - 1)) {
      __hip_atomic_store(h.ctr + tile_m, 0u, __ATOMIC_RELAXED, __HIP_MEMORY_SCOPE_AGENT);
      __hip_atomic_store(leave, 0u, __ATOMIC_RELAXED, __HIP_MEMORY_SCOPE_AGENT);
    }
  }
}

template <bool AKC, bool BKC, int NW = T32_NW, int NS = T32_NS, bool EARLY = false, bool REGU = false>
__global__ __launch_bounds__(NW * 64) void gemm_t32_kernel(T32Args g) {
  extern __shared__ __attribute__((aligned(1024))) float t32_smem[];
  gemm_t32_body<AKC, BKC, false, false, NW, NS, EARLY, REGU>(g, (int)blockIdx.x, t32_smem);
}

template <bool ARAG2>
__global__ __launch_bounds__(256) void gemm_t32_pair_kernel(T32Args g1, T32Args g2, int n1) {
  extern __shared__ __attribute__((aligned(1024))) float t32_smem[];
  if ((int)blockIdx.x < n1) gemm_t32_body<false, false, false>(g1, (int)blockIdx.x, t32_smem);
  else gemm_t32_body<false, false, ARAG2>(g2, (int)blockIdx.x - n1, t32_smem);
}

static bool t32_fill(const GemmProblem& p, T32Args& g, bool& akc, bool& bkc, bool allow_ragged_a = false, bool* ragged_a = nullptr) {
  if (p.dtype != TO_F32 || p.batch != 1 || p.reduce_batch) return false;
  if (p.loss_rows || p.tail_out || p.loss_out) return false;
  akc = p.a_sk == 1 && p.K > 1;
  bkc = p.b_sk == 1 && p.K > 1;
  if (!akc && p.a_sm != 1) return false;
  if (!bkc && p.b_sn != 1) return false;
  if (p.K % 4 != 0 || p.N % 4 != 0) return false;
  const bool rag = !akc && (p.M % 4 != 0 || p.a_sk % 4 != 0 || (reinterpret_cast<uintptr_t>(p.A) & 15u));
  if (ragged_a) *ragged_a = rag;
  if (rag && !allow_ragged_a) return false;
  if (akc && p.a_sm % 4 != 0) return false;
  if (bkc && p.b_sn % 4 != 0) return false;
  if (!bkc && p.b_sk % 4 != 0) return false;
  if ((reinterpret_cast<uintptr_t>(p.A) & 3u) || ((akc || !rag) && (reinterpret_cast<uintptr_t>(p.A) & 15u))) return false;
  if ((reinterpret_cast<uintptr_t>(p.B) | reinterpret_cast<uintptr_t>(p.C)) & 15u) return false;
  if (p.c_sm % 4 != 0) return false;
  if (p.Cin && (reinterpret_cast<uintptr_t>(p.Cin) & 15u)) return false;
  if (p.dact && (reinterpret_cast<uintptr_t>(p.dact) & 15u)) return false;
  if (p.bias && (reinterpret_cast<uintptr_t>(p.bias) & 15u)) return false;
  if (p.beta != 0.0 && !p.Cin) return false;
  if (p.act > 2) return false;
  if ((p.M + 32) * std::max<int64_t>(p.a_sm, 1) * 4 + p.K * std::max<int64_t>(p.a_sk, 1) * 4 >= (1LL << 31)) return false;
  if ((p.N + 32) * std::max<int64_t>(p.b_sn, 1) * 4 + p.K * std::max<int64_t>(p.b_sk, 1) * 4 >= (1LL << 31)) return false;
  g.A = (const float*)p.A; g.B = (const float*)p.B; g.C = (float*)p.C;
  g.Cin = p.beta != 0.0 ? (const float*)p.Cin : nullptr;
  g.M = (int)p.M; g.N = (int)p.N; g.K = (int)p.K;
  g.a_sx = akc ? p.a_sm : p.a_sk;
  g.b_sx = bkc ? p.b_sn : p.b_sk;
  g.c_sm = p.c_sm;
  g.tiles_m = (int)((p.M + 31) / 32); g.tiles_n = (int)((p.N + 31) / 32);
  {
    int best = 1 << 30;
    for (int gm : {8, 4, 2, 1}) {
      const int gn = 8 / gm;
      const int cost = (g.tiles_m + gm - 1) / gm + (g.tiles_n + gn - 1) / gn;
      if (cost < best) { best = cost; g.gm = gm; g.gn = gn; }
    }
  }
  g.alpha = (float)p.alpha; g.beta = (float)p.beta;
  g.bias = (const float*)p.bias; g.dact = (const float*)p.dact; g.act = p.act; g.dact_kind = p.dact_kind;
  g.rowsum = (float*)p.rowsum; g.rowsum_in = (const float*)p.rowsum_in; g.rowsum_alpha = (float)p.rowsum_alpha;
  g.rowsum_acc = p.rowsum_acc ? 1 : 0;
  static const int pd = [] { const char* e = ab_getenv("TOPS_T32_PD"); const int v = e ? atoi(e) : 2; return v < 1 ? 1 : (v > T32_NS ? T32_NS : v); }();
  g.pd = pd;
  static unsigned long long* dbg = [] {
    unsigned long long* p = nullptr;
    if (ab_getenv("TOPS_T32_STAMPS") && hipHostMalloc(reinterpret_cast<void**>(&p), 48 * sizeof(unsigned long long), hipHostMallocMapped) == hipSuccess) {
      for (int i = 0; i < 48; ++i) p[i] = 0;
      static unsigned long long* keep = p;
      atexit([] {
        if (keep[15]) {
          const unsigned long long* k = keep + 8;
          std::fprintf(stderr, "[t32] joined launch, workgroup 0, us since it began: its tile stored and arrived %.2f, all eight tiles of the row block "
                               "there %.2f, loss head of its four rows done %.2f, tail stored %.2f (entered %.2f us after stamp 0)\n",
                       (k[1] - k[0]) * 0.01, (k[2] - k[0]) * 0.01, (k[3] - k[0]) * 0.01, (k[4] - k[0]) * 0.01, ((double)k[0] - (double)keep[0]) * 0.01);
        }
        for (int w = 0; w < (keep[15] ? 1 : 2); ++w) {
          const unsigned long long* k = keep + 8 * w;
          std::fprintf(stderr, "[t32] %s workgroup of the last launch, us since it began: prologue DMA issued %.2f, first chunk landed %.2f, K loop done %.2f, "
                               "partials met %.2f, done %.2f; began %.2f us after workgroup 0\n", w ? "last" : "first",
                       (k[1] - k[0]) * 0.01, (k[2] - k[0]) * 0.01, (k[3] - k[0]) * 0.01, (k[4] - k[0]) * 0.01, (k[5] - k[0]) * 0.01,
                       ((double)k[0] - (double)keep[0]) * 0.01);
          const unsigned long long* wv = keep + 16 + 16 * w;
          std::fprintf(stderr, "[t32]   per wave, K loop done / partial written:");
          for (int q = 0; q < 8; ++q)
            if (wv[2 * q]) std::fprintf(stderr, "  w%d %.2f / %.2f", q, ((double)wv[2 * q] - (double)k[0]) * 0.01, ((double)wv[2 * q + 1] - (double)k[0]) * 0.01);
          std::fprintf(stderr, "\n");
        }
      });
    }
    return p;
  }();
  g.dbg = dbg;
  return true;
}

bool gemm_t32_applicable(const GemmProblem& p) {
  static const int enable = [] { const char* e = ab_getenv("TOPS_GEMM_T32"); return e ? atoi(e) : 1; }();
  if (!enable) return false;
  T32Args g;
  bool akc, bkc;
  if (!t32_fill(p, g, akc, bkc)) return false;
  const long tiles = (long)g.tiles_m * g.tiles_n;
  static const long max_tiles = [] { const char* e = ab_getenv("TOPS_T32_MAXTILES"); return e ? atol(e) : 512L; }();
  return tiles >= 96 && tiles <= max_tiles && p.K >= 256 && p.K <= 8192;
}

bool launch_gemm_t32_pair(const GemmProblem& p1, const GemmProblem& p2, hipStream_t s, bool dry);

static long t32_grid(const T32Args& g) {
  const long rm = (g.tiles_m + g.gm - 1) / g.gm, rn = (g.tiles_n + g.gn - 1) / g.gn;
  return 8 * rm * rn;
}

static void t32_attr(const void* k) { TO_HIP(hipFuncSetAttribute(k, hipFuncAttributeMaxDynamicSharedMemorySize, T32_NW * T32_WAVE * 4)); }

constexpr int T32_W8_DEFAULT = 1;
constexpr int T32_W8_NS = 1;
constexpr bool T32_EARLY = true;
constexpr bool T32_REGU = true;

template <int NW, int NS, bool EARLY, bool REGU = false>
static void t32_launch_nw(const T32Args& g, bool akc, bool bkc, hipStream_t s) {
  constexpr size_t lds = (size_t)NW * NS * T32_STAGE * 4;
  static bool attr = false;
  if (!attr) {
    TO_HIP(hipFuncSetAttribute(reinterpret_cast<const void*>(gemm_t32_kernel<true, true, NW, NS, EARLY, REGU>), hipFuncAttributeMaxDynamicSharedMemorySize, (int)lds));
    TO_HIP(hipFuncSetAttribute(reinterpret_cast<const void*>(gemm_t32_kernel<true, false, NW, NS, EARLY, REGU>), hipFuncAttributeMaxDynamicSharedMemorySize, (int)lds));
    TO_HIP(hipFuncSetAttribute(reinterpret_cast<const void*>(gemm_t32_kernel<false, true, NW, NS, EARLY, REGU>), hipFuncAttributeMaxDynamicSharedMemorySize, (int)lds));
    TO_HIP(hipFuncSetAttribute(reinterpret_cast<const void*>(gemm_t32_kernel<false, false, NW, NS, EARLY, REGU>), hipFuncAttributeMaxDynamicSharedMemorySize, (int)lds));
    attr = true;
  }
  const dim3 grid((unsigned)t32_grid(g)), block(NW * 64);
  if (akc && bkc) launch_k((gemm_t32_kernel<true, true, NW, NS, EARLY, REGU>), grid, block, lds, s, g);
  else if (akc) launch_k((gemm_t32_kernel<true, false, NW, NS, EARLY, REGU>), grid, block, lds, s, g);
  else if (bkc) launch_k((gemm_t32_kernel<false, true, NW, NS, EARLY, REGU>), grid, block, lds, s, g);
  else launch_k((gemm_t32_kernel<false, false, NW, NS, EARLY, REGU>), grid, block, lds, s, g);
}

void launch_gemm_t32(const GemmProblem& p, hipStream_t s) {
  T32Args g;
  bool akc, bkc;
  TO_CHECK(t32_fill(p, g, akc, bkc), TO_ERR_STATE, "launch_gemm_t32: not applicable");
  static const int cus = [] { hipDeviceProp_t pr; int d = 0; return (hipGetDevice(&d) == hipSuccess && hipGetDeviceProperties(&pr, d) == hipSuccess) ? pr.multiProcessorCount : 0; }();
  static const int waves = [] { const char* e = ab_getenv("TOPS_T32_WAVES"); return e ? atoi(e) : (T32_W8_DEFAULT ? 8 : 4); }();
  const bool w8 = waves == 8 && t32_grid(g) <= cus;
#ifdef TOPS_AB_KNOBS
  static const int w8_ns = [] { const char* e = ab_getenv("TOPS_T32_W8_NS"); return e ? atoi(e) : T32_W8_NS; }();
  static const int early = [] { const char* e = ab_getenv("TOPS_T32_EARLY"); return e ? atoi(e) : (int)T32_EARLY; }();
  static const int regu = [] { const char* e = ab_getenv("TOPS_T32_REGU"); return e ? atoi(e) : (int)T32_REGU; }();
  switch ((w8 ? (w8_ns == 1 ? 2 : 4) : 0) + (early ? 1 : 0)) {
    case 0: t32_launch_nw<T32_NW, T32_NS, false>(g, akc, bkc, s); break;
    case 1: t32_launch_nw<T32_NW, T32_NS, true>(g, akc, bkc, s); break;
    case 2: t32_launch_nw<8, 1, false>(g, akc, bkc, s); break;
    case 3:
      if (regu) t32_launch_nw<8, 1, true, true>(g, akc, bkc, s);
      else t32_launch_nw<8, 1, true, false>(g, akc, bkc, s);
      break;
    case 4: t32_launch_nw<8, 2, false>(g, akc, bkc, s); break;
    default: t32_launch_nw<8, 2, true>(g, akc, bkc, s); break;
  }
#else
  if (w8) t32_launch_nw<8, T32_W8_NS, T32_EARLY, T32_REGU>(g, akc, bkc, s);
  else t32_launch_nw<T32_NW, T32_NS, T32_EARLY>(g, akc, bkc, s);
#endif
  TO_HIP(hipGetLastError());
  count_launch();
}

static unsigned* g_t32_ctr = nullptr;
static int *g_t32_status = nullptr, *g_t32_status_dev = nullptr;
static bool g_t32_head_off = false;
void gemm_t32_init() {
  if (g_t32_ctr) return;
  if (hipMalloc(&g_t32_ctr, 2 * T32_CTR * sizeof(unsigned)) != hipSuccess || hipMemset(g_t32_ctr, 0, 2 * T32_CTR * sizeof(unsigned)) != hipSuccess) {
    (void)hipGetLastError();
    g_t32_ctr = nullptr;
    return;
  }
  if (hipHostMalloc(&g_t32_status, sizeof(int), hipHostMallocMapped) == hipSuccess) {
    *g_t32_status = 0;
    if (hipHostGetDevicePointer(reinterpret_cast<void**>(&g_t32_status_dev), g_t32_status, 0) != hipSuccess) g_t32_status_dev = nullptr;
  }
  (void)hipGetLastError();
}
int gemm_t32_take_failure() {
  const int st = g_t32_status ? *g_t32_status : 0;
  if (st) {
    g_t32_head_off = true;
    *g_t32_status = 0;
    if (g_t32_ctr) (void)hipMemset(g_t32_ctr, 0, 2 * T32_CTR * sizeof(unsigned));
  }
  return st;
}

bool launch_gemm_t32_head(const GemmProblem& pf, const GemmProblem& ph, hipStream_t s) {
  static const int enable = [] { const char* e = getenv("TOPS_STEP_SEAM"); return e ? atoi(e) : 0; }();
  if (enable != 3 || !g_t32_ctr || !g_t32_status_dev || g_t32_head_off) return false;
  T32Args g;
  bool akc, bkc;
  if (!t32_fill(pf, g, akc, bkc) || !akc || !bkc) return false;
  const long tiles = (long)g.tiles_m * g.tiles_n;
  if (tiles < 96 || tiles > 512 || pf.K < 256 || pf.K > 8192 || g.tiles_m > T32_CTR) return false;
  if (pf.act != 1 || pf.dact || pf.rowsum || pf.beta != 0.0) return false;
  if (pf.N != 256 || pf.c_sm != pf.N) return false;
  if (ph.dtype != TO_F32 || ph.batch != 1 || ph.reduce_batch) return false;
  if (ph.A != pf.C || ph.M != pf.M || ph.K != pf.N || ph.a_sk != 1 || ph.a_sm != pf.c_sm) return false;
  if (ph.b_sk != 1 || ph.b_sn % 4 != 0 || (reinterpret_cast<uintptr_t>(ph.B) & 15u)) return false;
  if (ph.N < 1 || ph.N > 16 || (ph.loss_rows != 1 && ph.loss_rows != 2) || !ph.target) return false;
  if (ph.beta != 0.0 || ph.dact || ph.act != 0 || ph.rowsum) return false;
  if (ph.tail_out) {
    if (ph.tail_kind) return false;
    if (ph.tail_n != pf.N || ph.tail_h != pf.C || ph.tail_w != ph.B || ph.b_sn != ph.tail_n) return false;
    if (reinterpret_cast<uintptr_t>(ph.tail_out) & 15u) return false;
  }
  g.gm = 8; g.gn = 1;
  if (g.tiles_m < 8) return false;
  {
    static const int cus = [] { hipDeviceProp_t pr; int d = 0; return (hipGetDevice(&d) == hipSuccess && hipGetDeviceProperties(&pr, d) == hipSuccess) ? pr.multiProcessorCount : 0; }();
    if (t32_grid(g) > cus) return false;
  }
  T32HeadArgs h{};
  h.W2 = (const float*)ph.B; h.bias2 = (const float*)ph.bias; h.target = (const float*)ph.target;
  h.dz = (float*)ph.C; h.loss_out = (float*)ph.loss_out; h.tail_out = (float*)ph.tail_out;
  h.ctr = g_t32_ctr;
  h.status = g_t32_status_dev;
  h.w_sn = ph.b_sn; h.dz_sm = ph.c_sm;
  h.N2 = (int)ph.N; h.loss_rows = ph.loss_rows; h.alpha2 = (float)ph.alpha;

  static bool attr = false;
  if (!attr) {
    TO_HIP(hipFuncSetAttribute(reinterpret_cast<const void*>(gemm_t32_head_kernel), hipFuncAttributeMaxDynamicSharedMemorySize, T32_NW * T32_WAVE * 4));
    attr = true;
  }
  launch_k(gemm_t32_head_kernel, dim3((unsigned)t32_grid(g)), dim3(256), (size_t)T32_NW * T32_WAVE * 4, s, g, h);
  TO_HIP(hipGetLastError());
  count_launch();
  return true;
}

bool launch_gemm_t32_pair(const GemmProblem& p1, const GemmProblem& p2, hipStream_t s, bool dry) {
  static const int enable = [] { const char* e = ab_getenv("TOPS_GEMM_T32_PAIR"); return e ? atoi(e) : 0; }();
  if (!enable) return false;
  T32Args g1, g2;
  bool akc1, bkc1, akc2, bkc2, rag2 = false;
  if (!t32_fill(p1, g1, akc1, bkc1) || akc1 || bkc1) return false;
  if (!t32_fill(p2, g2, akc2, bkc2, true, &rag2) || akc2 || bkc2) return false;
  const long n1 = (long)g1.tiles_m * g1.tiles_n, n2 = (long)g2.tiles_m * g2.tiles_n;
  if (n1 < 96 || n1 + n2 > 512 || p1.K < 256 || p1.K > 8192 || p2.K < 256 || p2.K > 8192 || n2 > n1) return false;
  if (dry) return true;
  static bool attr = false;
  if (!attr) {
    t32_attr(reinterpret_cast<const void*>(gemm_t32_pair_kernel<false>));
    t32_attr(reinterpret_cast<const void*>(gemm_t32_pair_kernel<true>));
    attr = true;
  }
  const long w1 = t32_grid(g1), w2 = t32_grid(g2);
  const dim3 grid((unsigned)(w1 + w2)), block(256);
  const size_t lds = (size_t)T32_NW * T32_WAVE * 4;
  if (rag2) launch_k(gemm_t32_pair_kernel<true>, grid, block, lds, s, g1, g2, (int)w1);
  else launch_k(gemm_t32_pair_kernel<false>, grid, block, lds, s, g1, g2, (int)w1);
  TO_HIP(hipGetLastError());
  count_launch();
  return true;
}

}
```

Measured before the change: 44410.

## Shorten kernel prologue: precomputed tile maps, narrowed strides, early operand loads

Reorders the kernel argument structs so the fields needed first sit together, and pins them into scalar registers at entry. Integer divisions in the tile mapping are replaced with host-precomputed magic multipliers and shifts. Strides are narrowed from 64-bit to 32-bit. The head kernel now issues its operand and tail loads before the epilogue prefetch, so memory latency starts earlier in these latency-bound small GEMMs. The risks are int overflow for large strides, wrong results if the magic-number division is off for some tile counts, and higher register pressure.

After: 46470 (median of 6 runs). 1.05x the previous value.

```diff
diff --git a/tensor-ops_amd/csrc/gemm_small.hip b/tensor-ops_amd/csrc/gemm_small.hip
--- a/tensor-ops_amd/csrc/gemm_small.hip
+++ b/tensor-ops_amd/csrc/gemm_small.hip
@@ -10,20 +10,22 @@
 struct SmallArgsT {
   const S* A;
   const S* B;
+  unsigned a_bytes, b_bytes;
+  int M, N, K;
+  int kper;
+  int tile_order;
+  unsigned map_d, map_mag, map_q, map_r;
+  int tiles_n;
+  int a_sm, a_sk, b_sk, b_sn;
+  int a_sb, b_sb;
   S* C;
   const S* Cin;
-  int M, N, K;
-  long a_sm, a_sk, b_sk, b_sn, c_sm;
-  long a_sb, b_sb, c_sb;
-  int a_vec, b_vec;
-  unsigned a_bytes, b_bytes;
-  int tiles_n;
-  int tiles_m;
-  int tile_order;
-  int kper;
-  S alpha, beta;
   const S* bias;
   const S* dact;
+  long c_sm, c_sb;
+  int a_vec, b_vec;
+  int tiles_m;
+  S alpha, beta;
   int act;
   int dact_kind;
   S* rowsum;
@@ -42,26 +44,37 @@
 #endif
 };
 
+template <bool EPI, class S>
+__device__ __forceinline__ void small_pin_hot(const SmallArgsT<S>& g) {
+  if constexpr (EPI) {
+    asm volatile("" ::"s"(g.M), "s"(g.N), "s"(g.tile_order), "s"(g.map_d), "s"(g.map_mag), "s"(g.map_q), "s"(g.map_r), "s"(g.Cin), "s"(g.bias),
+                 "s"(g.dact), "s"(g.c_sm));
+  } else {
+    asm volatile("" ::"s"(g.A), "s"(g.B), "s"(g.a_bytes), "s"(g.b_bytes), "s"(g.M), "s"(g.N), "s"(g.K), "s"(g.kper), "s"(g.tile_order),
+                 "s"(g.map_d), "s"(g.map_mag), "s"(g.map_q), "s"(g.map_r), "s"(g.tiles_n), "s"(g.a_sm), "s"(g.a_sk), "s"(g.b_sk), "s"(g.b_sn));
+  }
+}
+
 #ifdef TOPS_AB_KNOBS
+#define SM_STAMP_ON stamp_on
 #define SM_STAMP(i) do { if (stamp_on) g.dbg[i] = wall_clock64(); } while (0)
+#define SM_STAMP_ENTRY() do { stamp_on = g.dbg && bid == 0 && tid == 0; if (stamp_on) g.dbg[0] = t_entry; } while (0)
+#define SM_ENTRY_CLOCK() wall_clock64()
 #else
+#define SM_STAMP_ENTRY() do { } while (0)
+#define SM_ENTRY_CLOCK() 0ll
 #define SM_STAMP(i) do { } while (0)
 #endif
 
 
 template <class G>
 __device__ __forceinline__ void tile_of(const G& g, int bid, int& tile_m, int& tile_n) {
-  if (g.tile_order) {
-    const int T = g.tiles_m * g.tiles_n, x = bid & 7, q = T >> 3, r = T & 7;
-    bid = (x < r ? x * (q + 1) : r * (q + 1) + (x - r) * q) + (bid >> 3);
-  }
-  if (g.tile_order == 2) {
-    tile_n = bid / g.tiles_m;
-    tile_m = bid - tile_n * g.tiles_m;
-  } else {
-    tile_m = bid / g.tiles_n;
-    tile_n = bid - tile_m * g.tiles_n;
-  }
+  const unsigned x = (unsigned)bid & 7u;
+  const unsigned run = x * g.map_q + (x < g.map_r ? x : g.map_r) + ((unsigned)bid >> 3);
+  const unsigned t = g.tile_order ? run : (unsigned)bid;
+  const unsigned hi = g.map_d == 1u ? t : __umulhi(t, g.map_mag), lo = t - hi * g.map_d;
+  tile_m = (int)(g.tile_order == 2 ? lo : hi);
+  tile_n = (int)(g.tile_order == 2 ? hi : lo);
 }
 
 __device__ __forceinline__ float tanh_s(float x) { return tanhf(x); }
@@ -88,9 +101,15 @@
 template <int OFF>
 __device__ __forceinline__ double xor16(double x) { return __shfl_xor(x, OFF, 64); }
 
-template <class S, int AMODE, int BMODE, int NW, int TS, int ONESHOT = 0, bool EXT = false, int PARTS = 0, bool STAG = false, int TAILK = 0>
+template <class S, int AMODE, int BMODE, int NW, int TS, int ONESHOT = 0, bool EXT = false, int PARTS = 0, bool STAG = false, int TAILK = 0, bool HEAD = false, bool KMASK = false>
 __device__ __forceinline__ void gemm_small_body(const SmallArgsT<S>& g, const int bid, const long bz, S* ext_lds = nullptr,
-                                                const int tid_in = -1) {
+                                                const int tid_in = -1, const long long t_entry_in = 0, const bool have_entry = false) {
+#ifdef TOPS_AB_KNOBS
+  long long t_entry = have_entry ? t_entry_in : wall_clock64();
+  if (have_entry) asm volatile("" : "+v"(t_entry));
+  bool stamp_on = false;
+#endif
+  static_assert(!HEAD || (sizeof(S) == 4 && TS == 16 && ONESHOT && PARTS == 0), "HEAD: the fp32 16x16 one-shot in the compiler's order");
   constexpr int ES = (int)sizeof(S);
   static_assert(ES == 4 || TS == 16, "the fp64 matrix instruction is 16x16x4");
   constexpr int KG = (TS == 32) ? 2 : 4;
@@ -114,10 +133,6 @@
   }
   const int tid = tid_in >= 0 ? tid_in : (int)threadIdx.x, lane = tid & 63, wave = tid >> 6;
   const int l31 = lane & (TS - 1), half = lane / TS;
-#ifdef TOPS_AB_KNOBS
-  const bool stamp_on = g.dbg && bid == 0 && tid == 0;
-#endif
-  SM_STAMP(0);
   int tile_m, tile_n;
   tile_of(g, bid, tile_m, tile_n);
   const long m = (long)tile_m * TS + l31, n = (long)tile_n * TS + l31;
@@ -138,8 +153,8 @@
       const_cast<S*>(g.A), 0, g.a_bytes, 0x00020000);
   const __amdgpu_buffer_rsrc_t rb = __builtin_amdgcn_make_buffer_rsrc(
       const_cast<S*>(g.B), 0, g.b_bytes, 0x00020000);
-  const int a_base = (int)((bz * g.a_sb + (mv ? m : 0) * g.a_sm) * ES);
-  const int b_base = (int)((bz * g.b_sb + (nv ? n : 0) * g.b_sn) * ES);
+  const int a_base = (int)(((unsigned)bz * (unsigned)g.a_sb + (unsigned)(mv ? m : 0) * (unsigned)g.a_sm) * (unsigned)ES);
+  const int b_base = (int)(((unsigned)bz * (unsigned)g.b_sb + (unsigned)(nv ? n : 0) * (unsigned)g.b_sn) * (unsigned)ES);
   const int a_sk4 = (int)g.a_sk * ES, b_sk4 = (int)g.b_sk * ES;
   auto sel = [](bool ok, int off) { const int msk = -(int)ok; return (off & msk) | (0x7fffffff & ~msk); };
   typedef unsigned int u32x4 __attribute__((ext_vector_type(4)));
@@ -164,6 +179,16 @@
       d[2] = __hiloint2double((int)w.y, (int)w.x); d[3] = __hiloint2double((int)w.w, (int)w.z);
     }
   };
+  auto selk = [&](bool in, int k, int off) {
+    if constexpr (KMASK) {
+      int msk = (kend - 1 - k) >> 31;
+      asm("" : "+v"(msk));
+      msk |= -(int)!in;
+      return (off & ~msk) | (0x7fffffff & msk);
+    } else {
+      return sel(in & (k < kend), off);
+    }
+  };
   auto load_stage = [&](S (&a)[ST][4], S (&b)[ST][4], int k0) {
 #pragma unroll
     for (int c = 0; c < ST; ++c) {
@@ -172,13 +197,13 @@
         ld4(ra, mv & (kb < kend), a_base + kb * ES, a[c]);
       } else {
 #pragma unroll
-        for (int j = 0; j < 4; ++j) a[c][j] = ld1(ra, sel(mv & (kb + j < kend), a_base + (kb + j) * a_sk4));
+        for (int j = 0; j < 4; ++j) a[c][j] = ld1(ra, selk(mv, kb + j, a_base + (kb + j) * a_sk4));
       }
       if (BMODE == 1 && g.b_vec) {
         ld4(rb, nv & (kb < kend), b_base + kb * ES, b[c]);
       } else {
 #pragma unroll
-        for (int j = 0; j < 4; ++j) b[c][j] = ld1(rb, sel(nv & (kb + j < kend), b_base + (kb + j) * b_sk4));
+        for (int j = 0; j < 4; ++j) b[c][j] = ld1(rb, selk(nv, kb + j, b_base + (kb + j) * b_sk4));
       }
     }
   };
@@ -237,7 +262,7 @@
   const S* Ci = g.Cin ? g.Cin + bz * g.c_sb : nullptr;
   const S* Hd = g.dact ? g.dact + bz * g.c_sb : nullptr;
   S pf_ci[NRW], pf_hd[NRW], pf_bias = S(0);
-  {
+  auto prefetch_epilogue = [&] {
     const long col = (long)tile_n * TS + l31;
     if (g.bias && col < g.N) pf_bias = g.bias[col];
 #pragma unroll
@@ -249,15 +274,51 @@
       pf_ci[i] = (Ci && ok) ? Ci[row * g.c_sm + col] : S(0);
       pf_hd[i] = (Hd && ok) ? Hd[row * g.c_sm + col] : S(0);
     }
-  }
+  };
+  if constexpr (!HEAD) prefetch_epilogue();
   constexpr int SK = CK * ST;
-  SM_STAMP(1);
+  if constexpr (!HEAD) {
+    SM_STAMP_ENTRY();
+    SM_STAMP(1);
+  }
+  S tl_bw[2][4], tl_hv[2][4];
   if constexpr (ONESHOT) {
-    if constexpr (PARTS == 0) {
+    if constexpr (HEAD) {
+      load_stage(a0, b0, kbeg);
+      __builtin_amdgcn_sched_barrier(0);
+      {
+        const bool tl = g.loss_rows && g.tail_out;
+        const __amdgpu_buffer_rsrc_t rw = __builtin_amdgcn_make_buffer_rsrc(const_cast<S*>(g.tail_w), 0, tl ? g.N * g.tail_n * ES : 0, 0x00020000);
+        const __amdgpu_buffer_rsrc_t rh = __builtin_amdgcn_make_buffer_rsrc(const_cast<S*>(g.tail_h), 0, tl ? g.M * g.tail_n * ES : 0, 0x00020000);
+        const int kg = half, ntiles = (g.tail_n + 15) >> 4;
+#pragma unroll
+        for (int u = 0; u < 2; ++u) {
+          const int t = wave + u * NW, col = t * 16 + l31;
+          const bool cv = (t < ntiles) & (col < g.tail_n);
+#pragma unroll
+          for (int st = 0; st < 4; ++st) {
+            const int k = 4 * st + kg;
+            tl_bw[u][st] = ld1(rw, sel(cv & (k < g.N), (k * g.tail_n + col) * ES));
+          }
+#pragma unroll
+          for (int r = 0; r < 4; ++r) {
+            const int row = tile_m * 16 + row16(kg, r);
+            tl_hv[u][r] = ld1(rh, sel(cv & (row < g.M), (row * g.tail_n + col) * ES));
+          }
+        }
+      }
+      prefetch_epilogue();
+      __builtin_amdgcn_sched_barrier(0);
+      SM_STAMP_ENTRY();
+#ifdef TOPS_AB_KNOBS
+      if (SM_STAMP_ON) { SM_STAMP(2); __builtin_amdgcn_s_waitcnt(0x0F70); SM_STAMP(3); }
+#endif
+      mma_stage(a0, b0);
+    } else if constexpr (PARTS == 0) {
       if (kbeg < kend) {
         load_stage(a0, b0, kbeg);
 #ifdef TOPS_AB_KNOBS
-        if (stamp_on) { SM_STAMP(2); __builtin_amdgcn_s_waitcnt(0x0F70); SM_STAMP(3); }
+        if (SM_STAMP_ON) { SM_STAMP(2); __builtin_amdgcn_s_waitcnt(0x0F70); SM_STAMP(3); }
 #endif
         mma_stage(a0, b0);
       }
@@ -304,8 +365,7 @@
     }
   }
 
-  S tl_bw[2][4], tl_hv[2][4];
-  if constexpr (TS == 16) {
+  if constexpr (TS == 16 && !HEAD) {
     if (g.loss_rows && g.tail_out) {
       const int l15 = lane & 15, kg = lane >> 4;
       const int ntiles = (g.tail_n + 15) / 16;
@@ -439,7 +499,7 @@
     }
   }
 #ifdef TOPS_AB_KNOBS
-  if (stamp_on) { __builtin_amdgcn_s_waitcnt(0); SM_STAMP(8); }
+  if (SM_STAMP_ON) { __builtin_amdgcn_s_waitcnt(0); SM_STAMP(8); }
 #endif
 }
 
@@ -449,25 +509,32 @@
 }
 
 __global__ __launch_bounds__(8 * 64) void gemm_small_head_kernel(SmallArgsT<float> g) {
+  const long long t_entry = SM_ENTRY_CLOCK();
+  small_pin_hot<false>(g);
   g.a_vec = 1;
   g.b_vec = 1;
-  gemm_small_body<float, 0, 1, 8, 16, 2>(g, (int)blockIdx.x, (long)blockIdx.z);
+  gemm_small_body<float, 0, 1, 8, 16, 2, false, 0, false, 0, true>(g, (int)blockIdx.x, (long)blockIdx.z, nullptr, -1, t_entry, true);
 }
 __global__ __launch_bounds__(8 * 64) void gemm_small_head_tanh_kernel(SmallArgsT<float> g) {
+  const long long t_entry = SM_ENTRY_CLOCK();
+  small_pin_hot<false>(g);
   g.a_vec = 1;
   g.b_vec = 1;
-  gemm_small_body<float, 0, 1, 8, 16, 2, false, 0, false, ACT_KIND_TANH>(g, (int)blockIdx.x, (long)blockIdx.z);
+  gemm_small_body<float, 0, 1, 8, 16, 2, false, 0, false, ACT_KIND_TANH, true>(g, (int)blockIdx.x, (long)blockIdx.z, nullptr, -1, t_entry, true);
 }
 
 template <class S, int A1, int B1, int NW1, int TS1, int OS1, int A2, int B2, int NW2, int TS2, int OS2, int P1 = 0, bool STAG1 = false>
 __global__ __launch_bounds__((NW1 > NW2 ? NW1 : NW2) * 64) void gemm_small_pair_kernel(SmallArgsT<S> g1,
                                                                                          SmallArgsT<S> g2, int n1) {
-  if ((int)blockIdx.x < n1) {
+  const long long t_entry = SM_ENTRY_CLOCK();
+  asm volatile("" ::"s"(n1));
+  small_pin_hot<true>(g1);
+  if (__builtin_expect((int)blockIdx.x < n1, 1)) {
     if (NW1 < NW2 && (int)(threadIdx.x >> 6) >= NW1) return;
-    gemm_small_body<S, A1, B1, NW1, TS1, OS1, false, P1, STAG1>(g1, (int)blockIdx.x, 0);
+    gemm_small_body<S, A1, B1, NW1, TS1, OS1, false, P1, STAG1>(g1, (int)blockIdx.x, 0, nullptr, -1, t_entry, true);
   } else {
     if (NW2 < NW1 && (int)(threadIdx.x >> 6) >= NW2) return;
-    gemm_small_body<S, A2, B2, NW2, TS2, OS2>(g2, (int)blockIdx.x - n1, 0);
+    gemm_small_body<S, A2, B2, NW2, TS2, OS2, false, 0, false, 0, false, true>(g2, (int)blockIdx.x - n1, 0, nullptr, -1, t_entry, true);
   }
 }
 
@@ -624,8 +691,8 @@
   int a_base[2], b_base[2];
 #pragma unroll
   for (int h = 0; h < 2; ++h) {
-    a_base[h] = (int)((bz * g.a_sb + (mv[h] ? m[h] : 0) * g.a_sm) * 8);
-    b_base[h] = (int)((bz * g.b_sb + (nv[h] ? n[h] : 0) * g.b_sn) * 8);
+    a_base[h] = (int)(((unsigned)bz * (unsigned)g.a_sb + (unsigned)(mv[h] ? m[h] : 0) * (unsigned)g.a_sm) * 8u);
+    b_base[h] = (int)(((unsigned)bz * (unsigned)g.b_sb + (unsigned)(nv[h] ? n[h] : 0) * (unsigned)g.b_sn) * 8u);
   }
   const int a_sk8 = (int)g.a_sk * 8, b_sk8 = (int)g.b_sk * 8;
   auto sel = [](bool ok, int off) { const int msk = -(int)ok; return (off & msk) | (0x7fffffff & ~msk); };
@@ -802,6 +869,15 @@
   return col_cost < row_cost ? 2 : 1;
 }
 
+template <class S>
+static void small_plan_map(SmallArgsT<S>& g) {
+  const unsigned T = (unsigned)g.tiles_m * (unsigned)g.tiles_n;
+  g.map_q = T >> 3;
+  g.map_r = T & 7u;
+  g.map_d = (unsigned)(g.tile_order == 2 ? g.tiles_m : g.tiles_n);
+  g.map_mag = g.map_d >= 2u ? (unsigned)(0xFFFFFFFFull / g.map_d + 1ull) : 0u;
+}
+
 template <class S, int NW, int TS, int ONESHOT = 0, int TAILK = 0>
 static void launch_nw(SmallArgsT<S>& g, const GemmProblem& p, int amode, int bmode, hipStream_t s) {
   constexpr int CK = (TS == 32) ? 8 : 16;
@@ -811,6 +887,7 @@
   g.tiles_n = (int)((p.N + TS - 1) / TS);
   g.tiles_m = tiles_m;
   g.tile_order = pick_tile_order(p, TS, g.tiles_m, g.tiles_n);
+  small_plan_map(g);
   dim3 grid(tiles_m * g.tiles_n, 1, (unsigned)p.batch), block(NW * 64);
   switch (amode * 2 + bmode) {
     case 0: launch_k((gemm_small_kernel<S, 0, 0, NW, TS, ONESHOT, TAILK>), grid, block, 0, s, g); break;
@@ -832,7 +909,7 @@
     atexit([] {
       static const char* names[9] = {"entry", "set-up done", "operand batch issued", "operand batch landed", "MFMAs done, partial in LDS",
                                      "all partials there (barrier)", "reduced + epilogue / loss head, stores issued", "tail done", "stores acknowledged"};
-      std::fprintf(stderr, "[small stamps %d] tile 0, thread 0, us since its workgroup began:", want);
+      std::fprintf(stderr, "[small stamps %d] tile 0, thread 0, us since the first instruction of its kernel (a kernel that pins its argument block) or body:", want);
       for (int i = 1; i < 9; ++i)
         if (keep[i]) std::fprintf(stderr, "\n  %6.2f  %s", (keep[i] - keep[0]) * 0.01, names[i]);
       std::fprintf(stderr, "\n");
@@ -858,8 +935,8 @@
   g.A = (const S*)p.A; g.B = (const S*)p.B; g.C = (S*)p.C;
   g.Cin = (p.beta != 0.0) ? (const S*)p.Cin : nullptr;
   g.M = (int)p.M; g.N = (int)p.N; g.K = (int)p.K;
-  g.a_sm = p.a_sm; g.a_sk = p.a_sk; g.b_sk = p.b_sk; g.b_sn = p.b_sn; g.c_sm = p.c_sm;
-  g.a_sb = p.a_sb; g.b_sb = p.b_sb; g.c_sb = p.c_sb;
+  g.a_sm = (int)p.a_sm; g.a_sk = (int)p.a_sk; g.b_sk = (int)p.b_sk; g.b_sn = (int)p.b_sn; g.c_sm = p.c_sm;
+  g.a_sb = (int)p.a_sb; g.b_sb = (int)p.b_sb; g.c_sb = p.c_sb;
   g.alpha = (S)p.alpha; g.beta = (S)p.beta;
   g.bias = (const S*)p.bias; g.dact = (const S*)p.dact; g.act = p.act; g.dact_kind = p.dact_kind;
   g.rowsum = (S*)p.rowsum;
@@ -916,12 +993,14 @@
     g.tiles_n = (int)((p.N + 31) / 32);
     g.tiles_m = (int)((p.M + 31) / 32);
     g.tile_order = pick_tile_order(p, 32, g.tiles_m, g.tiles_n);
+    small_plan_map(g);
     return c;
   }
   g.kper = (int)(((chunks + c.nw - 1) / c.nw) * ck);
   g.tiles_n = (int)((p.N + c.ts - 1) / c.ts);
   g.tiles_m = (int)((p.M + c.ts - 1) / c.ts);
   g.tile_order = pick_tile_order(p, c.ts, g.tiles_m, g.tiles_n);
+  small_plan_map(g);
   return c;
 }
 
@@ -1122,9 +1201,11 @@
   if (ph.K > 8 * 2 * 16) return false;
   c.head.kper = (int)((((ph.K + 15) / 16 + 7) / 8) * 16);
   c.head.tile_order = 0;
+  small_plan_map(c.head);
   const int T = c.fwd.tiles_m * c.fwd.tiles_n;
   if (T % 8 != 0 || (T / 8) % c.fwd.tiles_n != 0 || c.fwd.tiles_m > 128) return false;
   c.fwd.tile_order = 1;
+  small_plan_map(c.fwd);
   if (!g_seam_ctr) return false;
   c.ctr = g_seam_ctr;
   c.mode = enable == 2 ? 2 : 1;
diff --git a/tensor-ops_amd/csrc/gemm_t32.hip b/tensor-ops_amd/csrc/gemm_t32.hip
--- a/tensor-ops_amd/csrc/gemm_t32.hip
+++ b/tensor-ops_amd/csrc/gemm_t32.hip
@@ -11,6 +11,12 @@
 struct T32Args {
   const float* A;
   const float* B;
+  long a_sx, b_sx;
+  int M, N, K;
+  int tiles_m, tiles_n;
+  int lgm, lgn;
+  unsigned wmag0, wmag1;
+  int pd;
   float* C;
   const float* Cin;
   const float* bias;
@@ -18,17 +24,18 @@
   float* rowsum;
   const float* rowsum_in;
   unsigned long long* dbg;
-  long a_sx, b_sx;
   long c_sm;
-  int M, N, K;
-  int tiles_m, tiles_n;
   int gm, gn;
   int act, dact_kind;
   int rowsum_acc;
-  int pd;
   float alpha, beta;
   float rowsum_alpha;
 };
+
+__device__ __forceinline__ void t32_pin_hot(const T32Args& g) {
+  asm volatile("" ::"s"(g.A), "s"(g.B), "s"(g.a_sx), "s"(g.b_sx), "s"(g.M), "s"(g.N), "s"(g.K), "s"(g.tiles_m), "s"(g.tiles_n),
+               "s"(g.lgm), "s"(g.lgn), "s"(g.wmag0), "s"(g.wmag1), "s"(g.pd));
+}
 
 __device__ __attribute__((aligned(16))) float g_t32_zero[4] = {0.f, 0.f, 0.f, 0.f};
 
@@ -37,13 +44,16 @@
 constexpr int T32_STAGE = 2 * 32 * T32_BK;
 constexpr int T32_WAVE = T32_NS * T32_STAGE;
 
-__device__ __forceinline__ bool t32_tile_of(int tiles_m, int tiles_n, int gm, int gn, int bid, int& tm, int& tn) {
-  const int x = bid & 7, local = bid >> 3, xm = x / gn, xn = x - xm * gn;
-  const int r0 = tiles_m * xm / gm, r1 = tiles_m * (xm + 1) / gm, c0 = tiles_n * xn / gn, c1 = tiles_n * (xn + 1) / gn;
+__device__ __forceinline__ bool t32_tile_of(const T32Args& g, int bid, int& tm, int& tn) {
+  const int x = bid & 7, local = bid >> 3, xm = x >> g.lgn, xn = x & ((1 << g.lgn) - 1);
+  const int r0 = (g.tiles_m * xm) >> g.lgm, r1 = (g.tiles_m * (xm + 1)) >> g.lgm;
+  const int c0 = (g.tiles_n * xn) >> g.lgn, c1 = (g.tiles_n * (xn + 1)) >> g.lgn;
   const int w = c1 - c0;
   if (w <= 0 || local >= (r1 - r0) * w) return false;
-  tm = r0 + local / w;
-  tn = c0 + local - (local / w) * w;
+  const unsigned mag = w == (g.tiles_n >> g.lgn) ? g.wmag0 : g.wmag1;
+  const int q = w == 1 ? local : (int)__umulhi((unsigned)local, mag);
+  tm = r0 + q;
+  tn = c0 + local - q * w;
   return true;
 }
 
@@ -56,20 +66,34 @@
   static_assert(WAVE_F >= 1024 + 64, "a wave's stage memory holds its partial tile and its row sums");
   static_assert(!ARAG || !AKC, "the dword form is for a row-contiguous A");
   constexpr int NA = ARAG ? 16 : 4, PER = NA + 4;
+#ifdef TOPS_AB_KNOBS
+  const unsigned long long t_entry = __builtin_amdgcn_s_memrealtime();
+#endif
+  t32_pin_hot(g);
   const int tid = threadIdx.x, lane = tid & 63;
   const int wave = __builtin_amdgcn_readfirstlane(tid >> 6);
   const int l31 = lane & 31, half = lane >> 5;
-  unsigned long long* const dbg = (g.dbg && tid == 0 && (bid == 0 || bid == (int)gridDim.x - 1)) ? g.dbg + (bid == 0 ? 0 : 8) : nullptr;
+#ifdef TOPS_AB_KNOBS
+  unsigned long long* dbg = nullptr;
+  unsigned long long* wdbg = nullptr;
   auto stamp = [&](int i) { if (dbg) dbg[i] = __builtin_amdgcn_s_memrealtime(); };
+  auto stamp_first = [&] {
+    const bool mine = g.dbg && (bid == 0 || bid == (int)gridDim.x - 1);
+    dbg = (mine && tid == 0) ? g.dbg + (bid == 0 ? 0 : 8) : nullptr;
+    wdbg = (mine && lane == 0 && wave < 8) ? g.dbg + 16 + (bid == 0 ? 0 : 16) + 2 * wave : nullptr;
+    if (dbg) { dbg[0] = t_entry; dbg[6] = __builtin_amdgcn_s_memrealtime(); }
+  };
+#else
+  auto stamp = [](int) {};
+  auto stamp_first = [] {};
+#endif
 #ifdef TOPS_AB_KNOBS
-  unsigned long long* const wdbg = (g.dbg && lane == 0 && wave < 8 && (bid == 0 || bid == (int)gridDim.x - 1)) ? g.dbg + 16 + (bid == 0 ? 0 : 16) + 2 * wave : nullptr;
 #define T32_WSTAMP(i) do { if (wdbg) wdbg[i] = __builtin_amdgcn_s_memrealtime(); } while (0)
 #else
 #define T32_WSTAMP(i) do { } while (0)
 #endif
   int tile_m, tile_n;
-  if (!t32_tile_of(g.tiles_m, g.tiles_n, g.gm, g.gn, bid, tile_m, tile_n)) return -1;
-  stamp(0);
+  if (!t32_tile_of(g, bid, tile_m, tile_n)) return -1;
   const int m0 = tile_m * 32, n0 = tile_n * 32;
 
   const int erow = tid >> 3, ec4 = (tid & 7) * 4;
@@ -86,8 +110,8 @@
   if constexpr (!EARLY) prefetch_epilogue();
 
   const int U = (g.K + 15) / 16;
-  const int k0 = (int)((long)U * wave / NW) * 16;
-  int k1 = (int)((long)U * (wave + 1) / NW) * 16;
+  const int k0 = (int)((unsigned)(U * wave) / (unsigned)NW) * 16;
+  int k1 = (int)((unsigned)(U * (wave + 1)) / (unsigned)NW) * 16;
   if (k1 > g.K) k1 = g.K;
   int kd = k1;
   bool ru = false;
@@ -187,7 +211,7 @@
 #pragma unroll
   for (int r = 0; r < 16; ++r) acc[r] = 0.f;
   float asum = 0.f;
-  const bool want_rs = g.rowsum != nullptr && tile_n == 0;
+  bool want_rs;
 
   const int PD = g.pd < NS ? g.pd : NS;
   const int pro = nC < PD ? nC : PD;
@@ -230,6 +254,8 @@
   if constexpr (EARLY) {
     if (pro > 0) issue(0);
     __builtin_amdgcn_sched_barrier(0);
+    stamp_first();
+    want_rs = g.rowsum != nullptr && tile_n == 0;
     if constexpr (REGU) {
       if (ru) {
         if (pro > 0) asm volatile("s_waitcnt vmcnt(%0)" ::"n"(PER) : "memory");
@@ -267,6 +293,8 @@
     for (int c = 1; c < pro; ++c) issue(c);
   } else {
     for (int c = 0; c < pro; ++c) issue(c);
+    stamp_first();
+    want_rs = g.rowsum != nullptr && tile_n == 0;
   }
   stamp(1);
 
@@ -400,7 +428,7 @@
   const int wave = __builtin_amdgcn_readfirstlane(tid >> 6);
   const unsigned long long t_entry = g.dbg ? __builtin_amdgcn_s_memrealtime() : 0ull;
   int tile_m, tile_n;
-  if (!t32_tile_of(g.tiles_m, g.tiles_n, g.gm, g.gn, (int)blockIdx.x, tile_m, tile_n)) return;
+  if (!t32_tile_of(g, (int)blockIdx.x, tile_m, tile_n)) return;
   const long grow = (long)tile_m * 32 + 4 * tile_n + wave;
   const bool rv = grow < g.M;
   f32x4 w4[16];
@@ -523,6 +551,18 @@
   extern __shared__ __attribute__((aligned(1024))) float t32_smem[];
   if ((int)blockIdx.x < n1) gemm_t32_body<false, false, false>(g1, (int)blockIdx.x, t32_smem);
   else gemm_t32_body<false, false, ARAG2>(g2, (int)blockIdx.x - n1, t32_smem);
+}
+
+static bool t32_plan_map(T32Args& g) {
+  if ((long)g.tiles_m * g.tiles_n > 65535) return false;
+  auto lg = [](int v) { int l = 0; while ((1 << l) < v) ++l; return l; };
+  auto mag = [](int w) { return w >= 2 ? (unsigned)((0xFFFFFFFFull / (unsigned)w) + 1ull) : 0u; };
+  g.lgm = lg(g.gm);
+  g.lgn = lg(g.gn);
+  const int wlo = g.tiles_n >> g.lgn;
+  g.wmag0 = mag(wlo);
+  g.wmag1 = mag(wlo + 1);
+  return true;
 }
 
 static bool t32_fill(const GemmProblem& p, T32Args& g, bool& akc, bool& bkc, bool allow_ragged_a = false, bool* ragged_a = nullptr) {
@@ -564,6 +604,7 @@
       if (cost < best) { best = cost; g.gm = gm; g.gn = gn; }
     }
   }
+  if (!t32_plan_map(g)) return false;
   g.alpha = (float)p.alpha; g.beta = (float)p.beta;
   g.bias = (const float*)p.bias; g.dact = (const float*)p.dact; g.act = p.act; g.dact_kind = p.dact_kind;
   g.rowsum = (float*)p.rowsum; g.rowsum_in = (const float*)p.rowsum_in; g.rowsum_alpha = (float)p.rowsum_alpha;
@@ -584,9 +625,9 @@
         }
         for (int w = 0; w < (keep[15] ? 1 : 2); ++w) {
           const unsigned long long* k = keep + 8 * w;
-          std::fprintf(stderr, "[t32] %s workgroup of the last launch, us since it began: prologue DMA issued %.2f, first chunk landed %.2f, K loop done %.2f, "
-                               "partials met %.2f, done %.2f; began %.2f us after workgroup 0\n", w ? "last" : "first",
-                       (k[1] - k[0]) * 0.01, (k[2] - k[0]) * 0.01, (k[3] - k[0]) * 0.01, (k[4] - k[0]) * 0.01, (k[5] - k[0]) * 0.01,
+          std::fprintf(stderr, "[t32] %s workgroup of the last launch, us since its first instruction: first operand load out %.2f, prologue DMA issued %.2f, "
+                               "first chunk landed %.2f, K loop done %.2f, partials met %.2f, done %.2f; began %.2f us after workgroup 0\n", w ? "last" : "first",
+                       (k[6] - k[0]) * 0.01, (k[1] - k[0]) * 0.01, (k[2] - k[0]) * 0.01, (k[3] - k[0]) * 0.01, (k[4] - k[0]) * 0.01, (k[5] - k[0]) * 0.01,
                        ((double)k[0] - (double)keep[0]) * 0.01);
           const unsigned long long* wv = keep + 16 + 16 * w;
           std::fprintf(stderr, "[t32]   per wave, K loop done / partial written:");
@@ -722,6 +763,7 @@
     if (reinterpret_cast<uintptr_t>(ph.tail_out) & 15u) return false;
   }
   g.gm = 8; g.gn = 1;
+  if (!t32_plan_map(g)) return false;
   if (g.tiles_m < 8) return false;
   {
     static const int cus = [] { hipDeviceProp_t pr; int d = 0; return (hipGetDevice(&d) == hipSuccess && hipGetDeviceProperties(&pr, d) == hipSuccess) ? pr.multiProcessorCount : 0; }();
```
